# Youncy-Hu/MAGE

Hardware: AMD Instinct MI355X
Metric: generated frames/sec (64x64, 16-frame clips) (higher is better)
Workload: dtype bf16

## Files before the change

### __graft_entry__.py

```python
import os
import subprocess
import sys

ROOT = os.path.dirname(os.path.abspath(__file__))
if ROOT not in sys.path:
    sys.path.insert(0, ROOT)


def build() -> None:
    env = dict(os.environ)
    env.setdefault("HIPCC", "/opt/rocm/bin/hipcc")
    subprocess.run(["make", "-C", os.path.join(ROOT, "mage_amd", "csrc"), "-j4"], check=True, env=env)
    subprocess.run(["make", "-C", os.path.join(ROOT, "mage_amd", "csrc"), "check4"], check=True, env=env)
    import mage_amd
    from mage_amd import _lib
    lib = _lib.load()
    assert lib.mage_abi_version() == _lib.ABI_VERSION


def smoke() -> None:
    import torch
    from mage_amd.utils import synth
    from mage_amd.utils.util import instantiate_from_config
    from oracle import mage_oracle as O

    assert torch.cuda.is_available(), "smoke() needs a GPU"
    L, B, seed = 4, 2, 21
    cfg = synth.mnist_model_config(frames_length=L)
    model = instantiate_from_config(cfg).eval()
    synth.fill_state_dict(model, seed)
    sd = {k: v.detach().clone() for k, v in model.state_dict().items()}
    batch = synth.synth_batch_mnist(B, L, seed=seed)
    model = model.to("cuda:0")
    video = model.autoregressive_generate({k: v.to("cuda:0") for k, v in batch.items()})
    torch.cuda.synchronize()
    want, want_tok, _, trace = O.mage_generate(sd, batch, L, return_trace=True)
    err = (video.cpu() - want).abs().max().item()
    got_tok = model.last_tokens.cpu()
    tok_ok = torch.equal(got_tok, want_tok)
    top2 = trace.topk(2, dim=-1)[0]
    margin = (top2[..., 0] - top2[..., 1]).abs()
    bad = got_tok != want_tok
    n_soft, n_hard = int((bad & (margin <= 2e-5)).sum()), int((bad & (margin > 2e-5)).sum())
    print(f"smoke: video {tuple(video.shape)} max|d| vs oracle {err:.2e}, tokens bit-exact: {tok_ok} "
          f"(soft flips inside 2e-5 margin: {n_soft}, hard mismatches: {n_hard}, min margin {margin.min().item():.2e})")
    assert err < 1e-4 and n_hard == 0 and n_soft == 0 and tok_ok, "smoke: the HIP path left the oracle's tokens / frames"
    with open("/proc/self/maps") as f:
        assert "libmage_hip.so" in f.read(), "native library not loaded"


if __name__ == "__main__":
    build()
    if "--smoke" in sys.argv:
        smoke()
```

### include/mage_hip.h

```cpp
#ifndef MAGE_HIP_H
#define MAGE_HIP_H

#include <stdint.h>

#ifdef __cplusplus
extern "C" {
#endif

#define MAGE_ABI_VERSION 10

enum { MAGE_F32 = 0, MAGE_BF16 = 1, MAGE_BF16X3 = 2, MAGE_F16X3 = 3, MAGE_F16 = 4 };
enum { MAGE_OK = 0, MAGE_EINVAL = -1, MAGE_EHIP = -2, MAGE_EUNSUPPORTED = -3 };
enum { MAGE_ACT_NONE = 0, MAGE_ACT_RELU = 1, MAGE_ACT_QUICKGELU = 2, MAGE_ACT_GELU_ERF = 3, MAGE_ACT_TANH = 4,
       MAGE_ACT_QUICKGELU_GRAD = 5  };

int mage_abi_version(void);
const char* mage_last_error(void);
int mage_init(int device);
int mage_check_device_errors(void* stream);

int mage_set_option(const char* name, int32_t value);
int mage_get_option(const char* name, int32_t* value);

typedef struct mage_gemm_desc {
    int32_t dtype;
    int32_t M, N, K;
    const void* A;
    const void* W;
    void* Y;
    int32_t lda, ldy;
    int32_t y_dtype;
    int32_t out_h, out_w, in_h, in_w;
    int32_t a_img_stride, a_off;
    int32_t taps_h, taps_w, cin, stride;
    int32_t dy0, dx0, dys, dxs;
    int32_t y_img_stride, y_mul_y, y_mul_x, y_off;
    const float* bias;
    const float* scale;
    const float* shift;
    int32_t act;
    const float* rowadd;
    int32_t rowadd_div, rowadd_mod;
    const void* residual;
    int32_t ldr, res_dtype;
    int32_t post_relu;
    int32_t ldw;
    int32_t n_split;
    int64_t a_split_stride, w_split_stride, y_split_stride;
    void* y2;
    int32_t ldy2;
    int32_t res_half;
    float* ln_part;
    const float* ln_stats;
    const float* ln_colsum;
    int32_t a_half;
    float ln_eps;
    const void* head_w;
    int32_t head_phases;
    int32_t a_relu;
    int64_t ln_part_rows;
} mage_gemm_desc;

int mage_gemm(const mage_gemm_desc* desc, void* stream);
int mage_gemm_kernel_name(const mage_gemm_desc* desc, char* buf, int32_t len);
int mage_gemm_is_small(int32_t M, int32_t N, int32_t K);
int mage_ln_stats(const float* part, int64_t rows, int32_t n_slices, int32_t C, float eps, float* stats, void* stream);
int mage_row_stats(const void* x, int32_t dtype, int64_t rows, int32_t C, int64_t ldx, float eps, float* stats, void* stream);

int mage_split(const float* x, int64_t ldx, void* y, int64_t ldy, int64_t rows, int32_t C, int32_t kind, void* stream);

int mage_split_rows(const float* x, int64_t ldx, void* y, int64_t rows, int32_t C, int32_t kind, int32_t relu, int64_t group,
                    int64_t group_stride, int64_t off, int64_t inner, int64_t inner_stride, float* x_relu, void* stream);

int mage_layernorm(const float* x, const float* gamma, const float* beta, void* y, int32_t y_dtype,
                   int64_t rows, int32_t C, float eps, void* stream);

typedef struct mage_attn_desc {
    int32_t dtype;
    const void* q;
    const void* k;
    const void* v;
    void* out;
    int32_t ldq, ldk, ldv, ldo;
    int32_t n_seq, inner;
    int32_t nq, nk, n_head;
    int32_t q_outer_stride, q_axis_stride;
    int32_t kv_outer_stride, kv_axis_stride;
    int32_t causal;
    const int32_t* kv_len;
    int32_t kv_len_div;
    float scale;
    int32_t out_split;
    float drop_p;
    uint64_t drop_seed;
    int32_t o_outer_stride, o_axis_stride;
} mage_attn_desc;

int mage_attention(const mage_attn_desc* desc, void* stream);

int mage_embedding(const int64_t* ids, const float* table, void* out, int32_t out_dtype, int64_t n,
                   int32_t C, int32_t n_table, int32_t relu, int64_t group, int64_t group_stride, int64_t off,
                   int64_t inner, int64_t inner_stride, void* stream);

int mage_table_conv(const int64_t* ids, int64_t n_img, int32_t H, int32_t W, int32_t taps_h, int32_t taps_w, const void* table,
                    int32_t table_dtype, int32_t n_codes, int32_t C, const float* pos, const float* bias, int32_t relu, const float* rowadd,
                    int64_t rowadd_div, int32_t rowadd_mod, void* y, int32_t y_dtype, int64_t ldy, int64_t group, int64_t y_group_stride,
                    int64_t y_off, void* stream);

int mage_resblock_table(const int64_t* ids, int64_t n_img, int32_t H, int32_t W, const void* table, int32_t n_codes, int32_t C,
                        const float* bias3, const float* codebook, const void* w1, const float* b1, const float* scale1, const float* shift1,
                        int32_t post_relu, void* y, int64_t ldy, int64_t y_img_stride, int64_t y_row_pitch, int64_t y_off, void* stream);

int mage_resblock_rows(const void* t, int64_t lda, const void* w1, const float* b1, const float* scale1, const float* shift1,
                       const void* residual, int64_t ldr, int32_t post_relu, void* y, int64_t ldy, int64_t n_img, int32_t H, int32_t W,
                       int32_t C, int64_t img_stride, int64_t row_pitch, int64_t off, void* stream);

int mage_vq_nearest(const float* z, const float* codebook_t, const float* c2, int64_t M, int32_t D, int32_t K,
                    int64_t* idx, float* margin, void* stream);
int mage_vq_prepare(const float* codebook, int32_t K, int32_t D, float* codebook_t, float* c2, void* stream);

int mage_argmax(const float* logits, int64_t rows, int32_t K, int64_t ld, int64_t group, int64_t in_group_stride,
                int64_t in_off, int64_t* out, int64_t out_group_stride, int64_t out_off, float* margin, void* stream);

#define MAGE_SAMPLE_MAX_K 4096
int mage_sample_tokens(const float* logits, int64_t rows, int32_t K, int64_t ld, int64_t group, int64_t in_group_stride,
                       int64_t in_off, int64_t* out, int64_t out_group_stride, int64_t out_off, const int64_t* seeds,
                       int64_t pos_off, float temperature, int32_t top_k, float top_p, void* stream);

int mage_token_logprob(const float* logits, int64_t rows, int32_t K, int64_t ld, int64_t group, int64_t in_group_stride, int64_t in_off,
                       const int64_t* tokens, float* logprob, int64_t tok_group_stride, int64_t tok_off, void* stream);

int mage_clip_scores(const float* logprob, int64_t n_clips, int32_t n_cand, int64_t per_clip, float* scores, int64_t* best, void* stream);

int mage_cross_entropy(const float* logits, const int64_t* target, int64_t rows, int32_t K, float* row_loss,
                       float* loss_mean, void* stream);

int mage_conv_in(const float* x, const float* weight_t, const float* bias, const float* scale, const float* shift,
                 void* y, int32_t y_dtype, int32_t N, int32_t cin, int32_t H, int32_t W, int32_t cout,
                 int32_t kh, int32_t kw, int32_t stride, int32_t pad, int32_t act, int32_t s2d, void* stream);
int mage_conv_out(const void* x, int32_t x_dtype, const float* weight_t, const float* bias, float* y,
                  int32_t N, int32_t IH, int32_t IW, int32_t cin, int32_t cout, int32_t transposed, void* stream);
int mage_convt_fold_tanh(const float* taps, const float* bias, float* y, int32_t N, int32_t IH, int32_t IW,
                         int32_t cout, void* stream);

int mage_maxpool2(const void* x, void* y, int32_t dtype, int32_t N, int32_t H, int32_t W, int32_t C, int32_t relu,
                  void* stream);
int mage_upsample2(const void* x, void* y, int32_t dtype, int32_t N, int32_t H, int32_t W, int32_t C, void* stream);
int mage_relu(const void* x, void* y, int32_t dtype, int64_t n, void* stream);
int mage_cast(const void* x, int32_t x_dtype, void* y, int32_t y_dtype, int64_t n, void* stream);

int mage_adain(const float* x, const float* gamma, const float* beta, float* out, int32_t B, int32_t P, int32_t C,
               float eps, void* stream);

int mage_add_scaled_rowvec(float* x, const float* s, const float* vec, int32_t B, int32_t P, int32_t C, void* stream);

int mage_row_affine(float* x, const float* rs, const float* table, int64_t rows, int32_t C, int32_t div, int32_t mod,
                    void* stream);

int mage_caption_mask(const int64_t* ids, int32_t B, int32_t S, int64_t padding_idx, int32_t* kv_len, float* keep, void* stream);
int mage_copy2d(void* dst, int64_t dst_pitch, const void* src, int64_t src_pitch, int64_t width_bytes, int64_t height, void* stream);

int mage_groupnorm_silu(const float* x, int64_t sample_stride_rows, int64_t row_off, int32_t n_samples, int32_t rows_per_sample,
                        int32_t C, int32_t groups, const float* gamma, const float* beta, float eps, float* stats, void* y,
                        int32_t y_dtype, void* stream);

int mage_groupnorm_act(const float* x, int64_t sample_stride_rows, int64_t row_off, int32_t n_samples, int32_t rows_per_sample,
                       int32_t C, int32_t groups, const float* gamma, const float* beta, float eps, float* stats,
                       const float* residual, int32_t act, void* y, int32_t y_dtype, int64_t y_sample_stride_rows,
                       int64_t y_row_off, void* stream);

int mage_reparam_kl(const float* mu, const float* logvar, const float* eps, float* out, float* kl_sum, int32_t B, int64_t n,
                    void* stream);

int mage_mse(const float* a, int64_t lda, const float* b, int64_t ldb, int64_t rows, int32_t cols, double* workspace, float* out,
             void* stream);



int mage_transpose(const void* x, int32_t dtype, int64_t ldx, void* y, int64_t ldy, int64_t y_row0, int64_t M, int64_t Mp, int32_t C,
                   int32_t out_h, int32_t out_w, int32_t in_h, int32_t in_w, int64_t img_stride, int64_t a_off, int32_t dy, int32_t dx,
                   int32_t stride, void* stream);
int mage_transpose_colsum(const void* x, int64_t ldx, void* y, int64_t ldy, int64_t M, int64_t Mp, int32_t C, int32_t out_w,
                          int64_t img_stride, int64_t a_off, float* colsum, int32_t n_part, void* stream);
int mage_gemm_tn(const void* dY, int64_t lda, const void* X, int64_t ldb, int64_t T, int32_t N, int32_t K, int32_t n_split,
                 int64_t tokens_per_split, float* partials, float* db_partials, void* stream);
int mage_colsum(const void* x, int64_t ld, int64_t T, int32_t C, float* partials, int32_t n_part, void* stream);
int mage_row_sum(const void* x, int32_t dtype, int64_t ld, int64_t n, int32_t rows, float* out, int32_t n_chunk, void* stream);
int mage_sum_partials(const float* part, int64_t stride, int32_t n_part, int64_t n, float* out, int32_t accumulate, void* stream);
int mage_layernorm_bwd(const float* x, const float* gamma, const void* dy, int32_t dy_dtype, float* dx, float* partials, int32_t n_part,
                       int64_t rows, int32_t C, float eps, int32_t accumulate, void* dx_bf16, float p, uint64_t seed, void* stream);
int mage_act(const void* x, void* y, int32_t dtype, int64_t n, int32_t act, void* stream);
int mage_act_bwd(const void* x, const void* dy, void* dx, int32_t dtype, int64_t n, int32_t act, void* stream);
int mage_cross_entropy_bwd(const float* logits, const int64_t* target, int64_t rows, int32_t K, const float* grad_out, void* dlogits,
                           int32_t dl_dtype, void* stream);
int mage_embedding_bwd(const int64_t* ids, const void* dout, int32_t dout_dtype, float* dtable, int64_t n, int32_t C, int32_t n_table,
                       int64_t padding_idx, int64_t group, int64_t group_stride, int64_t off, float* scratch, int64_t scratch_floats,
                       void* stream);
int mage_group_rowsum(const void* x, int32_t dtype, int64_t rows, int32_t C, int64_t div, int64_t mod, const float* row_scale,
                      int64_t row_scale_div, float* out, int32_t n_chunk, void* stream);
int mage_attention_bwd(const mage_attn_desc* desc, const void* dout, void* dq, void* dk, void* dv, int32_t ld_dq, int32_t ld_dk,
                       int32_t ld_dv, void* stream);
int mage_dropout(const void* x, int32_t x_dtype, void* y, int32_t y_dtype, int64_t n, float p, uint64_t seed, int32_t accumulate,
                 void* stream);
int mage_dropout_add(const void* x, int32_t x_dtype, const float* r, float* y, void* y_bf16, int64_t n, float p, uint64_t seed, void* stream);
int mage_dropout_add_layernorm(const void* x, int32_t x_dtype, const float* r, float* y, const float* gamma, const float* beta, void* yn,
                               int32_t yn_dtype, int64_t rows, int32_t C, float eps, float p, uint64_t seed, void* stream);
int mage_bn_colreduce(int32_t mode, const float* x, const float* dy, const float* mask, const float* mean, const float* rstd, int64_t rows,
                      int32_t C, float* partials, int32_t n_part, void* stream);
int mage_bn_apply(const float* x, const float* mean, const float* rstd, const float* gamma, const float* beta, const float* residual, void* y,
                  int32_t y_dtype, int64_t rows, int32_t C, int32_t relu, void* stream);
int mage_bn_bwd_apply(const float* x, const float* dy, const float* mask, const float* mean, const float* rstd, const float* gamma,
                      const float* sums, float* dx, int64_t rows, int32_t C, void* stream);
int mage_convt_unfold_tanh_bwd(const float* grad_y, const float* y, float* dtaps, int32_t N, int32_t IH, int32_t IW, int32_t cout, void* stream);
// ... 21 lines not shown
```

### mage_amd/_lib.py

```python
from __future__ import annotations

import ctypes as C
import os
from typing import Optional

_HERE = os.path.dirname(os.path.abspath(__file__))
LIB_PATH = os.environ.get("MAGE_HIP_LIB", os.path.join(_HERE, "lib", "libmage_hip.so"))

F32, BF16, BF16X3, F16X3, F16 = 0, 1, 2, 3, 4
ACT_NONE, ACT_RELU, ACT_QUICKGELU, ACT_GELU_ERF, ACT_TANH, ACT_QUICKGELU_GRAD = 0, 1, 2, 3, 4, 5
ABI_VERSION = 10

i32, i64, f32, vp = C.c_int32, C.c_int64, C.c_float, C.c_void_p


class GemmDesc(C.Structure):
    _fields_ = [
        ("dtype", i32), ("M", i32), ("N", i32), ("K", i32),
        ("A", vp), ("W", vp), ("Y", vp),
        ("lda", i32), ("ldy", i32), ("y_dtype", i32),
        ("out_h", i32), ("out_w", i32), ("in_h", i32), ("in_w", i32),
        ("a_img_stride", i32), ("a_off", i32),
        ("taps_h", i32), ("taps_w", i32), ("cin", i32), ("stride", i32),
        ("dy0", i32), ("dx0", i32), ("dys", i32), ("dxs", i32),
        ("y_img_stride", i32), ("y_mul_y", i32), ("y_mul_x", i32), ("y_off", i32),
        ("bias", vp), ("scale", vp), ("shift", vp),
        ("act", i32),
        ("rowadd", vp), ("rowadd_div", i32), ("rowadd_mod", i32),
        ("residual", vp), ("ldr", i32), ("res_dtype", i32),
        ("post_relu", i32), ("ldw", i32), ("n_split", i32),
        ("a_split_stride", i64), ("w_split_stride", i64), ("y_split_stride", i64),
        ("y2", vp), ("ldy2", i32), ("res_half", i32), ("ln_part", vp), ("ln_stats", vp), ("ln_colsum", vp), ("a_half", i32), ("ln_eps", C.c_float),
        ("head_w", vp), ("head_phases", i32), ("a_relu", i32), ("ln_part_rows", i64),
    ]


class AttnDesc(C.Structure):
    _fields_ = [
        ("dtype", i32), ("q", vp), ("k", vp), ("v", vp), ("out", vp),
        ("ldq", i32), ("ldk", i32), ("ldv", i32), ("ldo", i32),
        ("n_seq", i32), ("inner", i32), ("nq", i32), ("nk", i32), ("n_head", i32),
        ("q_outer_stride", i32), ("q_axis_stride", i32), ("kv_outer_stride", i32), ("kv_axis_stride", i32),
        ("causal", i32), ("kv_len", vp), ("kv_len_div", i32), ("scale", f32), ("out_split", i32), ("drop_p", f32), ("drop_seed", C.c_uint64),
        ("o_outer_stride", i32), ("o_axis_stride", i32),
    ]


SIGNATURES = {
    "mage_abi_version": (C.c_int, []),
    "mage_last_error": (C.c_char_p, []),
    "mage_init": (C.c_int, [C.c_int]),
    "mage_check_device_errors": (C.c_int, [vp]),
    "mage_set_option": (C.c_int, [C.c_char_p, i32]),
    "mage_get_option": (C.c_int, [C.c_char_p, C.POINTER(i32)]),
    "mage_gemm": (C.c_int, [C.POINTER(GemmDesc), vp]),
    "mage_gemm_kernel_name": (C.c_int, [C.POINTER(GemmDesc), C.c_char_p, i32]),
    "mage_gemm_is_small": (C.c_int, [i32, i32, i32]),
    "mage_ln_stats": (C.c_int, [vp, i64, i32, i32, f32, vp, vp]),
    "mage_row_stats": (C.c_int, [vp, i32, i64, i32, i64, f32, vp, vp]),
    "mage_groupnorm_bwd": (C.c_int, [vp, i64, i64, i32, i32, i32, i32, vp, vp, vp, vp, i32, vp, i64, i64, vp, vp, vp, vp, vp, vp]),
    "mage_adain_bwd": (C.c_int, [vp, vp, vp, vp, vp, i32, i32, i32, f32, vp]),
    "mage_reparam_kl_bwd": (C.c_int, [vp, vp, vp, vp, vp, vp, vp, i64, vp]),
    "mage_mse_bwd": (C.c_int, [vp, i64, vp, i64, i64, i32, vp, vp, i64, vp]),
    "mage_transpose_colsum": (C.c_int, [vp, i64, vp, i64, i64, i64, i32, i32, i64, i64, vp, i32, vp]),
    "mage_maxpool2_bwd": (C.c_int, [vp, vp, vp, i32, i32, i32, i32, vp]),
    "mage_upsample2_bwd": (C.c_int, [vp, vp, i32, i32, i32, i32, vp]),
    "mage_layernorm": (C.c_int, [vp, vp, vp, vp, i32, i64, i32, f32, vp]),
    "mage_split": (C.c_int, [vp, i64, vp, i64, i64, i32, i32, vp]),
    "mage_attention": (C.c_int, [C.POINTER(AttnDesc), vp]),
    "mage_embedding": (C.c_int, [vp, vp, vp, i32, i64, i32, i32, i32, i64, i64, i64, i64, i64, vp]),
    "mage_table_conv": (C.c_int, [vp, i64, i32, i32, i32, i32, vp, i32, i32, i32, vp, vp, i32, vp, i64, i32, vp, i32, i64, i64, i64, i64, vp]),
    "mage_resblock_table": (C.c_int, [vp, i64, i32, i32, vp, i32, i32, vp, vp, vp, vp, vp, vp, i32, vp, i64, i64, i64, i64, vp]),
    "mage_resblock_rows": (C.c_int, [vp, i64, vp, vp, vp, vp, vp, i64, i32, vp, i64, i64, i32, i32, i32, i64, i64, i64, vp]),
    "mage_vq_nearest": (C.c_int, [vp, vp, vp, i64, i32, i32, vp, vp, vp]),
    "mage_vq_prepare": (C.c_int, [vp, i32, i32, vp, vp, vp]),
    "mage_argmax": (C.c_int, [vp, i64, i32, i64, i64, i64, i64, vp, i64, i64, vp, vp]),
    "mage_sample_tokens": (C.c_int, [vp, i64, i32, i64, i64, i64, i64, vp, i64, i64, vp, i64, f32, i32, f32, vp]),
    "mage_token_logprob": (C.c_int, [vp, i64, i32, i64, i64, i64, i64, vp, vp, i64, i64, vp]),
    "mage_clip_scores": (C.c_int, [vp, i64, i32, i64, vp, vp, vp]),
    "mage_cross_entropy": (C.c_int, [vp, vp, i64, i32, vp, vp, vp]),
    "mage_conv_in": (C.c_int, [vp, vp, vp, vp, vp, vp, i32, i32, i32, i32, i32, i32, i32, i32, i32, i32, i32, i32, vp]),
    "mage_split_rows": (C.c_int, [vp, i64, vp, i64, i32, i32, i32, i64, i64, i64, i64, i64, vp, vp]),
    "mage_conv_out": (C.c_int, [vp, i32, vp, vp, vp, i32, i32, i32, i32, i32, i32, vp]),
    "mage_convt_fold_tanh": (C.c_int, [vp, vp, vp, i32, i32, i32, i32, vp]),
    "mage_maxpool2": (C.c_int, [vp, vp, i32, i32, i32, i32, i32, i32, vp]),
    "mage_upsample2": (C.c_int, [vp, vp, i32, i32, i32, i32, i32, vp]),
    "mage_relu": (C.c_int, [vp, vp, i32, i64, vp]),
    "mage_cast": (C.c_int, [vp, i32, vp, i32, i64, vp]),
    "mage_adain": (C.c_int, [vp, vp, vp, vp, i32, i32, i32, f32, vp]),
    "mage_add_scaled_rowvec": (C.c_int, [vp, vp, vp, i32, i32, i32, vp]),
    "mage_row_affine": (C.c_int, [vp, vp, vp, i64, i32, i32, i32, vp]),
    "mage_caption_mask": (C.c_int, [vp, i32, i32, i64, vp, vp, vp]),
    "mage_copy2d": (C.c_int, [vp, i64, vp, i64, i64, i64, vp]),
    "mage_groupnorm_silu": (C.c_int, [vp, i64, i64, i32, i32, i32, i32, vp, vp, f32, vp, vp, i32, vp]),
    "mage_groupnorm_act": (C.c_int, [vp, i64, i64, i32, i32, i32, i32, vp, vp, f32, vp, vp, i32, vp, i32, i64, i64, vp]),
    "mage_reparam_kl": (C.c_int, [vp, vp, vp, vp, vp, i32, i64, vp]),
    "mage_mse": (C.c_int, [vp, i64, vp, i64, i64, i32, vp, vp, vp]),
    "mage_transpose": (C.c_int, [vp, i32, i64, vp, i64, i64, i64, i64, i32, i32, i32, i32, i32, i64, i64, i32, i32, i32, vp]),
    "mage_bn_colreduce": (C.c_int, [i32, vp, vp, vp, vp, vp, i64, i32, vp, i32, vp]),
    "mage_bn_apply": (C.c_int, [vp, vp, vp, vp, vp, vp, vp, i32, i64, i32, i32, vp]),
    "mage_bn_bwd_apply": (C.c_int, [vp, vp, vp, vp, vp, vp, vp, vp, i64, i32, vp]),
    "mage_convt_unfold_tanh_bwd": (C.c_int, [vp, vp, vp, i32, i32, i32, i32, vp]),
    "mage_gemm_tn": (C.c_int, [vp, i64, vp, i64, i64, i32, i32, i32, i64, vp, vp, vp]),
    "mage_colsum": (C.c_int, [vp, i64, i64, i32, vp, i32, vp]),
    "mage_row_sum": (C.c_int, [vp, i32, i64, i64, i32, vp, i32, vp]),
    "mage_sum_partials": (C.c_int, [vp, i64, i32, i64, vp, i32, vp]),
    "mage_layernorm_bwd": (C.c_int, [vp, vp, vp, i32, vp, vp, i32, i64, i32, f32, i32, vp, f32, C.c_uint64, vp]),
    "mage_act": (C.c_int, [vp, vp, i32, i64, i32, vp]),
    "mage_act_bwd": (C.c_int, [vp, vp, vp, i32, i64, i32, vp]),
    "mage_cross_entropy_bwd": (C.c_int, [vp, vp, i64, i32, vp, vp, i32, vp]),
    "mage_embedding_bwd": (C.c_int, [vp, vp, i32, vp, i64, i32, i32, i64, i64, i64, i64, vp, i64, vp]),
    "mage_group_rowsum": (C.c_int, [vp, i32, i64, i32, i64, i64, vp, i64, vp, i32, vp]),
    "mage_attention_bwd": (C.c_int, [C.POINTER(AttnDesc), vp, vp, vp, vp, i32, i32, i32, vp]),
    "mage_dropout": (C.c_int, [vp, i32, vp, i32, i64, f32, C.c_uint64, i32, vp]),
    "mage_dropout_add": (C.c_int, [vp, i32, vp, vp, vp, i64, f32, C.c_uint64, vp]),
    "mage_dropout_add_layernorm": (C.c_int, [vp, i32, vp, vp, vp, vp, vp, i32, i64, i32, f32, f32, C.c_uint64, vp]),
    "mage_adam": (C.c_int, [vp, vp, vp, vp, i64, f32, f32, f32, f32, i32, f32, vp]),
}

_lib: Optional[C.CDLL] = None
_inited_devices = set()


class MageHipError(RuntimeError):
    pass


def load(path: str = LIB_PATH) -> C.CDLL:
    global _lib
    if _lib is not None:
        return _lib
    if not os.path.exists(path):
        raise MageHipError(
            f"{path} not found: the HIP extension is not built. Run `python -c 'import __graft_entry__ as g; g.build()'` "
            f"(or `make -C mage_amd/csrc`). There is no CPU/PyTorch fallback for the MAGE product path.")
    import torch
    lib = C.CDLL(path)
    for name, (res, args) in SIGNATURES.items():
        fn = getattr(lib, name)
        fn.restype, fn.argtypes = res, args
    if lib.mage_abi_version() != ABI_VERSION:
        raise MageHipError(f"libmage_hip.so ABI {lib.mage_abi_version()} != binding ABI {ABI_VERSION}: rebuild")
    _lib = lib
    return lib


def lib(device_index: int = 0) -> C.CDLL:
    l = load()
    if device_index not in _inited_devices:
        check(l.mage_init(int(device_index)), l)
        _inited_devices.add(device_index)
    return l


def check(code: int, l: Optional[C.CDLL] = None) -> None:
    if code == 0:
        return
    l = l or load()
    msg = (l.mage_last_error() or b"").decode(errors="replace")
    if code == -1:
        raise ValueError(f"mage_hip: {msg}")
    raise MageHipError(f"mage_hip error {code}: {msg}")
```

### mage_amd/config.py

```python
from __future__ import annotations

import contextlib
import dataclasses
import os
from typing import Iterator

__all__ = ["Config", "ENV", "get", "override", "lib_option", "lib_options", "lib_flag", "LIB_OPTIONS"]


@dataclasses.dataclass(frozen=True)
class Config:
    ln_fold: bool = True
    stream_16bit: bool = True
    attn_split: bool = True
    frame_table: bool = True
    auto_graph: bool = True
    encode_split: bool = True
    decode_table: bool = True
    decode_split: bool = True
    decode_taps8: bool = True
    decode_resblock_fusion: bool = True
    decode_head_fusion: bool = True
    decode_phase_merge: bool = True
    decode_relu_fold: bool = True
    train_f32_branch: bool = False
    train_wgrad_transpose: bool = False
    train_emit: bool = True
    train_dual: bool = True
    train_taps: bool = True
    train_enc_split: bool = True


ENV = {
    "ln_fold": ("MAGE_NO_LN_FOLD", False),
    "stream_16bit": ("MAGE_STREAM_FP32", False),
    "attn_split": ("MAGE_ATTN_SPLIT_FP32", False),
    "frame_table": ("MAGE_NO_FRAME_TABLE", False),
    "auto_graph": ("MAGE_NO_AUTO_GRAPH", False),
    "encode_split": ("MAGE_ENCODE_FP32", False),
    "decode_table": ("MAGE_NO_DECODE_TABLE", False),
    "decode_split": ("MAGE_DECODE_FP32", False),
    "decode_taps8": ("MAGE_DECODE_NO_TAPS8", False),
    "decode_resblock_fusion": ("MAGE_DECODE_NO_RESBLOCK_FUSION", False),
    "decode_head_fusion": ("MAGE_DECODE_NO_HEAD_FUSION", False),
    "decode_phase_merge": ("MAGE_DECODE_NO_PHASE_MERGE", False),
    "decode_relu_fold": ("MAGE_DECODE_NO_RELU_FOLD", False),
    "train_f32_branch": ("MAGE_TRAIN_F32_BRANCH", True),
    "train_wgrad_transpose": ("MAGE_WGRAD_TRANSPOSE", True),
    "train_emit": ("MAGE_TRAIN_NO_EMIT", False),
    "train_dual": ("MAGE_TRAIN_NO_DUAL", False),
    "train_taps": ("MAGE_TRAIN_NO_TAPS", False),
    "train_enc_split": ("MAGE_TRAIN_ENC_FP32", False),
}

LIB_OPTIONS = ("gemm_no_4w", "gemm_no_4h", "gemm_4h_plain", "gemm4_train_forms", "gemm_no_8phase", "gemm_no_taps8", "gemm_no_narrow", "gemm_no_narrow_few", "gemm_no_small",
               "gemm_small_m", "gemm_stagger_groups", "gemm_stagger_percent", "gemm_stagger_forced",
               "gemm4_stagger_groups", "gemm4_stagger_percent", "attn_no_mfma", "attn_no_fewq", "vq_no_mfma", "conv_no_tile")


def _set(v) -> bool:
    return bool(v) and v != "0"


def _from_env() -> Config:
    kw = {}
    for field, (var, when_set) in ENV.items():
        if _set(os.environ.get(var)):
            kw[field] = when_set
    return Config(**kw)


_CONFIG = _from_env()


def get() -> Config:
    return _CONFIG


@contextlib.contextmanager
def override(**kw) -> Iterator[Config]:
    global _CONFIG
    saved = _CONFIG
    _CONFIG = dataclasses.replace(saved, **kw)
    try:
        yield _CONFIG
    finally:
        _CONFIG = saved


_LIB_CACHE = None


def invalidate_lib_options() -> None:
    global _LIB_CACHE
    _LIB_CACHE = None


def _lib_cache() -> dict:
    global _LIB_CACHE
    if _LIB_CACHE is None:
        import ctypes as C
        from . import _lib
        l = _lib.load()
        out = {}
        for name in LIB_OPTIONS:
            v = C.c_int32(0)
            _lib.check(l.mage_get_option(name.encode(), C.byref(v)), l)
            out[name] = int(v.value)
        _LIB_CACHE = out
    return _LIB_CACHE


def lib_options() -> dict:
    return dict(_lib_cache())


def lib_flag(name: str) -> int:
    c = _lib_cache()
    if name not in c:
        raise KeyError(f"unknown library option '{name}' (mage_amd.config.LIB_OPTIONS)")
    return c[name]


def set_lib_option(name: str, value: int) -> None:
    from . import _lib
    l = _lib.load()
    try:
        _lib.check(l.mage_set_option(name.encode(), int(value)), l)
    finally:
        invalidate_lib_options()


@contextlib.contextmanager
def lib_option(name: str, value: int) -> Iterator[None]:
    old = lib_flag(name)
    set_lib_option(name, value)
    try:
        yield
    finally:
        set_lib_option(name, old)
```

### mage_amd/csrc/common.h

```cpp
#pragma once
#include <hip/hip_runtime.h>
#include <stdint.h>
#include <stdio.h>
#include <stdarg.h>
#include "../../include/mage_hip.h"

typedef __bf16 bf16_t;
typedef __attribute__((ext_vector_type(8))) __bf16 bf16x8;
typedef __attribute__((ext_vector_type(4))) __bf16 bf16x4;
typedef __attribute__((ext_vector_type(4))) float f32x4;
typedef __attribute__((ext_vector_type(4))) unsigned int u32x4;

#define MAGE_MAX_DEVICES 16
void mage_set_error(const char* fmt, ...);
int mage_device_index();
const void* mage_zero_page();
int* mage_error_word();
enum { MAGE_DEVERR_EMBEDDING_ID = 1, MAGE_DEVERR_CE_TARGET = 2, MAGE_DEVERR_TOKEN_ID = 3 };
struct MageOptions {
    int gemm_no_4w;
    int gemm_no_4h;
    int gemm_4h_plain;
    int gemm4_train_forms;
    int gemm_no_8phase;
    int gemm_no_taps8;
    int gemm_no_narrow;
    int gemm_no_narrow_few;
    int gemm_no_small;
    int gemm_small_m;
    int gemm_stagger_groups, gemm_stagger_percent, gemm_stagger_forced;
    int gemm4_stagger_groups, gemm4_stagger_percent;
    int attn_no_mfma;
    int attn_no_fewq;
    int vq_no_mfma;
    int conv_no_tile;
};
const MageOptions& mage_options();
__device__ __forceinline__ void mage_raise(int* word, int code, long value, int bound) {
    if (atomicCAS(word, 0, code) == 0) {
        word[1] = (int)value;
        word[2] = bound;
    }
}

#if defined(MAGE_DEBUG) && MAGE_DEBUG
#include <cassert>
#define MAGE_DASSERT(cond) assert(cond)
#else
#define MAGE_DASSERT(cond) ((void)0)
#endif

#define MAGE_CHECK_ARG(cond, ...)                                   \
    do {                                                            \
        if (!(cond)) {                                              \
            mage_set_error(__VA_ARGS__);                            \
            return MAGE_EINVAL;                                     \
        }                                                           \
    } while (0)

#define MAGE_CHECK_LAUNCH(name)                                                         \
    do {                                                                                \
        hipError_t e_ = hipGetLastError();                                              \
        if (e_ != hipSuccess) {                                                         \
            mage_set_error("%s: launch failed: %s", name, hipGetErrorString(e_));       \
            return MAGE_EHIP;                                                           \
        }                                                                               \
    } while (0)

int mage_gemm_cu_count();
extern thread_local const void** mage_gemm_plan;
template <auto KERNEL, typename Args>
int mage_gemm_launch(unsigned grid, unsigned block, unsigned lds, hipStream_t s, const Args& a) {
    if (mage_gemm_plan) {
        *mage_gemm_plan = (const void*)KERNEL;
        return MAGE_OK;
    }
    static bool attr[MAGE_MAX_DEVICES] = {false};
    const int dev = mage_device_index();
    MAGE_CHECK_ARG(dev >= 0, "mage_gemm: no current device");
    if (!attr[dev]) {
        (void)hipFuncSetAttribute((const void*)KERNEL, hipFuncAttributeMaxDynamicSharedMemorySize, lds);
        attr[dev] = true;
    }
    hipLaunchKernelGGL(KERNEL, dim3(grid), dim3(block), lds, s, a);
    MAGE_CHECK_LAUNCH("mage_gemm");
    return MAGE_OK;
}

__device__ __forceinline__ unsigned short f2bf_bits(float f) {
    unsigned int u = __float_as_uint(f);
    if ((u & 0x7fffffffu) > 0x7f800000u) return (unsigned short)((u >> 16) | 0x40);
    u += 0x7fffu + ((u >> 16) & 1u);
    return (unsigned short)(u >> 16);
}
__device__ __forceinline__ float bf_bits2f(unsigned short b) { return __uint_as_float(((unsigned int)b) << 16); }

template <typename T> __device__ __forceinline__ float to_f32(T v);
template <> __device__ __forceinline__ float to_f32<float>(float v) { return v; }
template <> __device__ __forceinline__ float to_f32<unsigned short>(unsigned short v) { return bf_bits2f(v); }

template <typename T> __device__ __forceinline__ T from_f32(float v);
template <> __device__ __forceinline__ float from_f32<float>(float v) { return v; }
template <> __device__ __forceinline__ unsigned short from_f32<unsigned short>(float v) { return f2bf_bits(v); }

typedef _Float16 f16_t;
template <> __device__ __forceinline__ float to_f32<f16_t>(f16_t v) { return (float)v; }
template <> __device__ __forceinline__ f16_t from_f32<f16_t>(float v) { return (f16_t)v; }

__device__ __forceinline__ f32x4 load4(const float* p) { return *(const f32x4*)p; }
__device__ __forceinline__ f32x4 load4(const unsigned short* p) {
    uint2 r = *(const uint2*)p;
    f32x4 o;
    o[0] = __uint_as_float(r.x << 16);
    o[1] = __uint_as_float(r.x & 0xffff0000u);
    o[2] = __uint_as_float(r.y << 16);
    o[3] = __uint_as_float(r.y & 0xffff0000u);
    return o;
}
__device__ __forceinline__ void store4(float* p, f32x4 v) { *(f32x4*)p = v; }
__device__ __forceinline__ void mage_ln_stats_row(const float2* __restrict__ p, long stride, int n_slices, float inv_c, float eps, float& mean, float& rstd) {
    float s1 = 0.f, s2 = 0.f;
    for (int i = 0; i < n_slices; ++i) {
        const float2 v = p[(long)i * stride];
        s1 = __fadd_rn(s1, v.x);
        s2 = __fadd_rn(s2, v.y);
    }
    mean = __fmul_rn(s1, inv_c);
    const float var = fmaxf(__fmaf_rn(-mean, mean, __fmul_rn(s2, inv_c)), 0.f);
    rstd = __fdiv_rn(1.0f, __fsqrt_rn(__fadd_rn(var, eps)));
}

typedef __attribute__((ext_vector_type(2))) __bf16 bf16x2_t;
__device__ __forceinline__ unsigned int pack_bf16x2(float a, float b) {
    bf16x2_t v = {(__bf16)a, (__bf16)b};
    return __builtin_bit_cast(unsigned int, v);
}
__device__ __forceinline__ void store4(unsigned short* p, f32x4 v) {
    uint2 r;
    r.x = pack_bf16x2(v[0], v[1]);
    r.y = pack_bf16x2(v[2], v[3]);
    *(uint2*)p = r;
}

__device__ __forceinline__ void store8(unsigned short* p, f32x4 a, f32x4 b) {
    uint4 r;
    r.x = pack_bf16x2(a[0], a[1]);
    r.y = pack_bf16x2(a[2], a[3]);
    r.z = pack_bf16x2(b[0], b[1]);
    r.w = pack_bf16x2(b[2], b[3]);
    *(uint4*)p = r;
}
__device__ __forceinline__ void store8(float* p, f32x4 a, f32x4 b) { *(f32x4*)p = a; *(f32x4*)(p + 4) = b; }

typedef __attribute__((ext_vector_type(2))) _Float16 f16x2_t;
typedef __attribute__((ext_vector_type(8))) _Float16 f16x8;
__device__ __forceinline__ unsigned int pack_f16x2(float a, float b) {
    const f16x2_t v = {(_Float16)a, (_Float16)b};
    return __builtin_bit_cast(unsigned int, v);
}
__device__ __forceinline__ float2 unpack_f16x2(unsigned int u) {
    const f16x2_t v = __builtin_bit_cast(f16x2_t, u);
    return float2{(float)v[0], (float)v[1]};
}
__device__ __forceinline__ float2 unpack_bf16x2(unsigned int u) { return float2{__uint_as_float(u << 16), __uint_as_float(u & 0xffff0000u)}; }
template <typename T> __device__ __forceinline__ unsigned int pack16x2(float a, float b) {
    if constexpr (sizeof(T) == 2 && !__is_same(T, unsigned short)) return pack_f16x2(a, b);
    else return pack_bf16x2(a, b);
}
template <typename T> __device__ __forceinline__ float2 unpack16x2(unsigned int u) {
    if constexpr (sizeof(T) == 2 && !__is_same(T, unsigned short)) return unpack_f16x2(u);
    else return unpack_bf16x2(u);
}
template <typename T> __device__ __forceinline__ f32x4 widen4(uint2 r) {
    const float2 a = unpack16x2<T>(r.x), b = unpack16x2<T>(r.y);
    return f32x4{a.x, a.y, b.x, b.y};
}
template <typename T> __device__ __forceinline__ f32x4 mfma16x16x32(const u32x4& a, const u32x4& b, const f32x4& c) {
    if constexpr (sizeof(T) == 2 && !__is_same(T, unsigned short))
        return __builtin_amdgcn_mfma_f32_16x16x32_f16(__builtin_bit_cast(f16x8, a), __builtin_bit_cast(f16x8, b), c, 0, 0, 0);
    else
        return __builtin_amdgcn_mfma_f32_16x16x32_bf16(__builtin_bit_cast(bf16x8, a), __builtin_bit_cast(bf16x8, b), c, 0, 0, 0);
}
__device__ __forceinline__ f32x4 load4(const f16_t* p) { return widen4<f16_t>(*(const uint2*)p); }
__device__ __forceinline__ void store4(f16_t* p, f32x4 v) { *(uint2*)p = uint2{pack_f16x2(v[0], v[1]), pack_f16x2(v[2], v[3])}; }
__device__ __forceinline__ void store8(f16_t* p, f32x4 a, f32x4 b) {
    *(uint4*)p = uint4{pack_f16x2(a[0], a[1]), pack_f16x2(a[2], a[3]), pack_f16x2(b[0], b[1]), pack_f16x2(b[2], b[3])};
// ... 72 lines not shown
```

### mage_amd/csrc/gemm.hip

```cpp
#include <cxxabi.h>
#include <cstring>
#include <mutex>
#include <string>
#include <unordered_map>
#include "gemm_impl.h"

int mage_gemm_f16(const mage_gemm_desc* d, hipStream_t s);

#ifdef MAGE_PROBE
extern "C" int mage_debug_read_waves(void* dst, size_t bytes) {
    return hipMemcpyFromSymbol(dst, HIP_SYMBOL(mage_probe_wave), bytes < sizeof(mage_probe_wave) ? bytes : sizeof(mage_probe_wave)) ==
                   hipSuccess
               ? 0
               : -1;
}
extern "C" int mage_debug_read_seg(void* dst, size_t bytes) {
    return hipMemcpyFromSymbol(dst, HIP_SYMBOL(mage_probe_seg), bytes < sizeof(mage_probe_seg) ? bytes : sizeof(mage_probe_seg)) ==
                   hipSuccess
               ? 0
               : -1;
}
extern "C" int mage_debug_read(void* dst, size_t bytes) {
    return hipMemcpyFromSymbol(dst, HIP_SYMBOL(mage_probe_buf), bytes < sizeof(mage_probe_buf) ? bytes : sizeof(mage_probe_buf)) ==
                   hipSuccess
               ? 0
               : -1;
}
#endif


extern "C" int mage_gemm_is_small(int32_t M, int32_t N, int32_t K) {
    MAGE_CHECK_ARG(mage_device_index() >= 0 && M > 0 && N > 0 && K > 0, "mage_gemm_is_small: no current device / bad sizes");
    return small_shape(M, N, K, mage_gemm_cu_count()) ? 1 : 0;
}

extern "C" int mage_gemm(const mage_gemm_desc* d_in, void* stream) {
    MAGE_CHECK_ARG(d_in != nullptr, "mage_gemm: null descriptor");
    mage_gemm_desc dn = *d_in;
    const bool spl = dn.dtype == MAGE_BF16X3 || dn.dtype == MAGE_F16X3;
    if (dn.ldw == 0) dn.ldw = spl ? 2 * dn.K : dn.K;
    if (dn.n_split <= 0) dn.n_split = 1;
    const mage_gemm_desc* d = &dn;
    MAGE_CHECK_ARG(d->ldw >= (spl ? 2 * d->K : d->K), "mage_gemm: ldw=%d < K=%d", d->ldw, d->K);
    MAGE_CHECK_ARG(d->ldw == d->K || d->n_split > 1 || spl,
                   "mage_gemm: ldw=%d != K=%d: a W row stride other than K is read only by the split-K (n_split > 1) and split-precision forms", d->ldw, d->K);
    MAGE_CHECK_ARG(mage_zero_page() != nullptr, "mage_gemm: mage_init() has not been called");
    const bool h16 = d->dtype == MAGE_F16;
    MAGE_CHECK_ARG(d->dtype == MAGE_F32 || d->dtype == MAGE_BF16 || h16 || spl, "mage_gemm: bad dtype %d", d->dtype);
    MAGE_CHECK_ARG(d->y_dtype == MAGE_F32 || (d->y_dtype == MAGE_BF16 && !h16) || ((spl || h16) && d->y_dtype == d->dtype),
                   "mage_gemm: bad y_dtype %d for dtype %d (fp32, or the operands' 16-bit / split type; fp32 operands may write bf16)", d->y_dtype, d->dtype);
    MAGE_CHECK_ARG(!d->residual || d->res_dtype == MAGE_F32 || (d->res_dtype == MAGE_BF16 && !h16) || (h16 && d->res_dtype == MAGE_F16),
                   "mage_gemm: bad res_dtype %d for dtype %d", d->res_dtype, d->dtype);
    MAGE_CHECK_ARG(!spl || (d->K % 64 == 0 && d->cin % 64 == 0 && d->lda >= 2 * d->cin && d->y_dtype != MAGE_BF16),
                   "mage_gemm: split-precision operands need K and cin multiples of 64, lda >= 2 cin (16-bit elements), fp32 or split output");
    MAGE_CHECK_ARG(!spl || d->y_dtype == MAGE_F32 || (d->N % 64 == 0 && d->ldy % 8 == 0 && d->ldy >= 2 * d->N && (((uintptr_t)d->Y) & 255) == 0),
                   "mage_gemm: split output needs N %% 64 == 0, ldy >= 2N (16-bit elements), Y 256-byte aligned");
    MAGE_CHECK_ARG(d->M > 0 && d->N > 0 && d->K > 0, "mage_gemm: empty problem M=%d N=%d K=%d", d->M, d->N, d->K);
    MAGE_CHECK_ARG(d->A && d->W && d->Y, "mage_gemm: null operand");
    const int ch = d->dtype == MAGE_F32 ? 4 : 8;
    MAGE_CHECK_ARG(d->N % 8 == 0, "mage_gemm: N=%d must be a multiple of 8", d->N);
    MAGE_CHECK_ARG(d->K % ch == 0 && d->lda % ch == 0 && d->cin % ch == 0,
                   "mage_gemm: K=%d, lda=%d, cin=%d must be multiples of %d", d->K, d->lda, d->cin, ch);
    MAGE_CHECK_ARG(d->ldy % 4 == 0 && (!d->residual || d->ldr % 4 == 0), "mage_gemm: ldy/ldr must be multiples of 4");
    MAGE_CHECK_ARG((d->y_dtype != MAGE_BF16 && d->y_dtype != MAGE_F16) || d->ldy % 8 == 0, "mage_gemm: 16-bit output needs ldy a multiple of 8 (16-byte accesses)");
    MAGE_CHECK_ARG(!d->residual || d->res_dtype == MAGE_F32 || d->ldr % 8 == 0, "mage_gemm: a 16-bit residual needs ldr a multiple of 8 (16-byte accesses)");
    MAGE_CHECK_ARG(d->taps_h >= 1 && d->taps_w >= 1 && d->K == d->taps_h * d->taps_w * d->cin,
                   "mage_gemm: K=%d != taps_h*taps_w*cin = %d*%d*%d", d->K, d->taps_h, d->taps_w, d->cin);
    MAGE_CHECK_ARG(d->out_h >= 1 && d->out_w >= 1 && d->in_h >= 1 && d->in_w >= 1, "mage_gemm: bad geometry");
    MAGE_CHECK_ARG(!d->scale == !d->shift, "mage_gemm: scale and shift must be given together");
    MAGE_CHECK_ARG(!d->rowadd || (d->rowadd_div >= 1 && d->rowadd_mod >= 1), "mage_gemm: bad rowadd div/mod");
    MAGE_CHECK_ARG((((uintptr_t)d->A | (uintptr_t)d->W | (uintptr_t)d->Y) & 15) == 0, "mage_gemm: operands must be 16-byte aligned");
    const bool gather_ = d->taps_h * d->taps_w > 1 || d->stride != 1 || d->dy0 != 0 || d->dx0 != 0 || d->in_h != d->out_h || d->in_w != d->out_w;
    MAGE_CHECK_ARG(d->n_split == 1 || (!gather_ && !d->residual && !d->rowadd && !d->scale && !d->post_relu && !d->bias &&
                                       d->out_h == 1 && d->out_w >= d->M && d->act == MAGE_ACT_NONE),
                   "mage_gemm: n_split > 1 is the plain split-K form (no gather, no epilogue extras, rows not regrouped)");
    MAGE_CHECK_ARG(d->n_split == 1 || ((d->a_split_stride | d->w_split_stride) % ch == 0 && d->y_split_stride % 4 == 0 && d->ldw % ch == 0),
                   "mage_gemm: split strides / ldw must keep 16-byte alignment");
    hipStream_t s = (hipStream_t)stream;
    MAGE_CHECK_ARG(!d->a_half || (d->in_h % 2 == 0 && d->in_w % 2 == 0 && d->n_split == 1), "mage_gemm: a_half needs an even in_h x in_w grid");
    MAGE_CHECK_ARG(!d->res_half || (d->residual && d->out_h > 1 && d->out_h % 2 == 0 && d->out_w % 2 == 0 && d->n_split == 1),
                   "mage_gemm: res_half needs a residual and an even out_h x out_w output plane");
    MAGE_CHECK_ARG(!d->ln_part || d->ln_part_rows > (d->ln_colsum ? (int64_t)d->M - 1 : (int64_t)(d->M - 1) * d->y_mul_x + d->y_off),
                   "mage_gemm: ln_part needs ln_part_rows (rows of the slice-major partial-sum buffer) > the largest row it is indexed with");
    MAGE_CHECK_ARG(!d->a_relu || (d->dtype == MAGE_BF16 && !gather_ && !d->a_half && d->N <= 128 && d->n_split == 1 && !d->residual && !d->rowadd && !d->scale &&
                                  !d->post_relu && !d->y2 && !d->ln_part && !d->ln_stats && !d->ln_colsum && !d->head_w),
                   "mage_gemm: a_relu is a form of the bf16 plain GEMM with N <= 128 (epilogue act(acc + bias) only)");
    if (spl) {
        const bool tapsform = gather_ || d->rowadd;
        MAGE_CHECK_ARG(!d->head_w, "mage_gemm: head_w is a fusion of the bf16 padded-taps form");
        if (tapsform) {
            const int r = d->dtype == MAGE_BF16X3 ? try_taps8<1>(d, s) : try_taps8<2>(d, s);
            if (r) return r < 0 ? r : MAGE_OK;
            mage_set_error("mage_gemm: split-precision form: this convolution / row-table geometry is not eligible for the padded-taps kernel");
            return MAGE_EUNSUPPORTED;
        }
        return d->dtype == MAGE_BF16X3 ? launch_spl<1>(d, s) : launch_spl<2>(d, s);
    }
    if (h16) {
        MAGE_CHECK_ARG(!d->head_w && d->n_split == 1 && !d->scale && !d->post_relu && !d->res_half && !d->a_half,
                       "mage_gemm: MAGE_F16 operands do not take head_w / n_split / scale+shift / post_relu / res_half / a_half");
        return mage_gemm_f16(d, s);
    }
    if (const int r = try_taps8(d, s)) return r < 0 ? r : MAGE_OK;
    MAGE_CHECK_ARG(!d->head_w, "mage_gemm: head_w is a fusion of the bf16 padded-taps form; this geometry does not run there");
    if (const int r = mage_conv3x3_c64_try(d, s)) return r < 0 ? r : MAGE_OK;
    if (const int r = mage_gemm4_try(d, s)) return r < 0 ? r : MAGE_OK;
    const bool gather = d->taps_h * d->taps_w > 1 || d->stride != 1 || d->dy0 != 0 || d->dx0 != 0 || d->in_h != d->out_h ||
                        d->in_w != d->out_w || d->a_half;
    if (d->dtype == MAGE_BF16) return gather ? launch<MAGE_BF16, true>(d, s) : launch<MAGE_BF16, false>(d, s);
    return gather ? launch<MAGE_F32, true>(d, s) : launch<MAGE_F32, false>(d, s);
}

thread_local const void** mage_gemm_plan = nullptr;

extern "C" int mage_gemm_kernel_name(const mage_gemm_desc* desc, char* buf, int32_t len) {
    MAGE_CHECK_ARG(buf != nullptr && len > 0, "mage_gemm_kernel_name: no buffer");
    const void* kernel = nullptr;
    mage_gemm_plan = &kernel;
    const int r = mage_gemm(desc, nullptr);
    mage_gemm_plan = nullptr;
    if (r != MAGE_OK) return r;
    static std::mutex mu;
    static std::unordered_map<const void*, std::string> names;
    std::string name;
    {
        std::lock_guard<std::mutex> lock(mu);
        auto it = names.find(kernel);
        if (it == names.end()) {
            hipFunction_t f = nullptr;
            const char* raw = hipGetFuncBySymbol(&f, kernel) == hipSuccess ? hipKernelNameRef(f) : nullptr;
            if (!raw) {
                mage_set_error("mage_gemm_kernel_name: the runtime has no name for the selected kernel");
                return MAGE_EHIP;
            }
            std::string n = raw;
            int status = -1;
            if (char* dm = n.compare(0, 2, "_Z") == 0 ? abi::__cxa_demangle(raw, nullptr, nullptr, &status) : nullptr) {
                if (status == 0) n = dm;
                free(dm);
            }
            for (const char* drop : {"void ", "(anonymous namespace)::"})
                for (size_t at; (at = n.find(drop)) != std::string::npos;) n.erase(at, strlen(drop));
            n = n.substr(0, n.find('('));
            it = names.emplace(kernel, n).first;
        }
        name = it->second;
    }
    MAGE_CHECK_ARG((int32_t)name.size() < len, "mage_gemm_kernel_name: %d bytes are too few for '%s'", (int)len, name.c_str());
    memcpy(buf, name.c_str(), name.size() + 1);
    return MAGE_OK;
}
```

### mage_amd/csrc/gemm_shared.h

```cpp
#pragma once
#include <type_traits>
#include "common.h"

namespace {

__device__ __forceinline__ void glds16(const void* src, char* lds_wave_base) {
    __builtin_amdgcn_global_load_lds((const __attribute__((address_space(1))) void*)src,
                                     (__attribute__((address_space(3))) void*)lds_wave_base, 16, 0, 0);
}

template <int ACT>
__device__ __forceinline__ float act_apply(float v) {
    if (ACT == MAGE_ACT_RELU) return fmaxf(v, 0.f);
    if (ACT == MAGE_ACT_QUICKGELU) return v * __builtin_amdgcn_rcpf(1.f + __builtin_amdgcn_exp2f(-2.4554669596f * v));
    if (ACT == MAGE_ACT_GELU_ERF) return 0.5f * v * (1.f + erff(v * 0.70710678118654752f));
    return v;
}

enum { EK_BIAS = 0, EK_RES_INIT = 1, EK_GENERAL = 2 };

struct LnConsume {
    float mean[8], rstd[8];
    f32x4 s[4];
};
enum { LN_NONE = 0, LN_PRODUCE = 1, LN_CONSUME = 2, LN_DUAL = 3, LN_GELUBWD = 4, LN_HEAD = 5 };

template <int ACT, typename OT, int MT, bool AFFINE = false, int LN = LN_NONE, int OSPL = 0,
          typename HT = std::conditional_t<sizeof(OT) == 2, OT, unsigned short>, bool RESE = false>
__device__ __forceinline__ void epilogue_lean(const mage_gemm_desc& d, const f32x4 (&bias)[4], f32x4 (&acc)[MT][4], int m0, int n0,
                                              int lane, int plane, char* stg, long ysplit, const LnConsume* lnc = nullptr) {
    constexpr bool F32 = sizeof(OT) == 4;
    static_assert((LN != LN_DUAL && LN != LN_GELUBWD) || std::is_same<HT, unsigned short>::value, "training forms: bf16 rows");
    static_assert(!RESE || (sizeof(OT) == 2 && OSPL == 0 && (LN == LN_NONE || LN == LN_PRODUCE)), "residual in the epilogue: 16-bit rows out");
    constexpr int RB = F32 ? 256 : 128;
    constexpr int NCH = RB / 16;
    constexpr int RPI = 64 / NCH;
    constexpr int NST = 16 / RPI;
    constexpr int CPC = 16 / (int)sizeof(OT);
    const int l15 = lane & 15, grp = lane >> 4;
    int woff[4];
#pragma unroll
    for (int nt = 0; nt < 4; ++nt)
        woff[nt] = OSPL ? l15 * RB + (((nt * 2 + (grp >> 1)) ^ l15) << 4) + (grp & 1) * 8
                 : F32  ? l15 * RB + (((nt * 4 + grp) ^ l15) << 4)
                        : l15 * RB + (((nt * 2 + (grp >> 1)) ^ ((l15 >> 1) & 7)) << 4) + (grp & 1) * 8;
    const int rr = lane / NCH, cc = lane % NCH;
    int roff[NST];
#pragma unroll
    for (int i = 0; i < NST; ++i) {
        const int r = rr + RPI * i;
        roff[i] = F32 ? r * RB + ((cc ^ r) << 4) : r * RB + ((cc ^ ((r >> 1) & 7)) << 4);
    }
    const int col = n0 + cc * CPC;
#pragma unroll
    for (int nt = 0; nt < 4; ++nt)
        MAGE_DASSERT(woff[nt] >= 0 && (OSPL ? (woff[nt] | 128) + 8 : woff[nt] + (F32 ? 16 : 8)) <= 4096);
#pragma unroll
    for (int i = 0; i < NST; ++i) MAGE_DASSERT(roff[i] >= 0 && roff[i] + 16 <= 4096);
    const bool simple_rows = d.out_h == 1 && d.out_w >= d.M;
    const bool affine_rows = AFFINE && d.out_h == 1 && d.y_mul_x == 1 && d.out_w % 256 == 0;
    const bool interior = (simple_rows || affine_rows) && m0 + MT * 16 <= d.M && n0 + 64 <= d.N;
    const bool cv_ok = col < d.N;
    const long row_shift = (AFFINE && !simple_rows && affine_rows) ? (long)(m0 / d.out_w) * (d.y_img_stride - d.out_w) : 0;
    const int ldy = OSPL ? d.ldy >> 1 : d.ldy;
    OT* yp = (OT*)d.Y + ysplit + ((long)((m0 + rr) * d.y_mul_x + d.y_off) + row_shift) * ldy + col;
    const long step = (long)RPI * d.y_mul_x * ldy;
    [[maybe_unused]] HT* y2p = nullptr;
    [[maybe_unused]] long step2 = 0;
    if constexpr (LN == LN_PRODUCE) {
        y2p = (HT*)d.y2 + (long)((m0 + rr) * d.y_mul_x + d.y_off) * d.ldy2 + col;
        step2 = (long)RPI * d.y_mul_x * d.ldy2;
    }

    [[maybe_unused]] u32x4 auxr[2][2];
    [[maybe_unused]] auto aux_request = [&](int mt) {
        const unsigned short* ap = (const unsigned short*)d.y2 + (long)((m0 + mt * 16 + (lane >> 3)) * d.y_mul_x + d.y_off) * d.ldy2 + n0 + (lane & 7) * 8;
#pragma unroll
        for (int i = 0; i < 2; ++i) auxr[mt & 1][i] = *(const u32x4*)(ap + (long)(8 * i) * d.y_mul_x * d.ldy2);
    };
    if constexpr (LN == LN_GELUBWD) aux_request(0);
    constexpr int RD = 3;
    [[maybe_unused]] u32x4 rland[RESE ? RD : 1][2];
    [[maybe_unused]] const HT* rbase = nullptr;
    [[maybe_unused]] auto res_request = [&](int t) {
#pragma unroll
        for (int i = 0; i < 2; ++i) {
            const int m = min(m0 + t * 16 + (lane >> 3) + 8 * i, d.M - 1);
            if constexpr (AFFINE) {
                const int img = m / plane, rem = m - img * plane;
                const int oy = rem / d.out_w, ox = rem - oy * d.out_w;
                const long rrow = d.res_half ? (long)img * (plane >> 2) + (long)(oy >> 1) * (d.out_w >> 1) + (ox >> 1) : (long)m;
                rland[t % RD][i] = *(const u32x4*)(rbase + rrow * d.ldr);
            } else {
                rland[t % RD][i] = *(const u32x4*)(rbase + (long)(m * d.y_mul_x + d.y_off) * d.ldr);
            }
        }
    };
    if constexpr (RESE) {
        const int rcol = n0 + (lane & 7) * 8;
        rbase = (const HT*)d.residual + (rcol < d.N ? rcol : 0);
#pragma unroll
        for (int t = 0; t < RD && t < MT; ++t) res_request(t);
    }
    auto stage = [&](int mt, u32x4 (&o)[NST], auto apply_act) {
        [[maybe_unused]] float s1 = 0.f, s2 = 0.f;
        [[maybe_unused]] uint2 auxb[4];
        if constexpr (RESE) {
#pragma unroll
            for (int i = 0; i < 2; ++i) {
                const int r = (lane >> 3) + 8 * i;
                *(u32x4*)(stg + 2048 + r * 128 + (((lane & 7) ^ ((r >> 1) & 7)) << 4)) = rland[mt % RD][i];
            }
            if (mt + RD < MT) res_request(mt + RD);
#pragma unroll
            for (int nt = 0; nt < 4; ++nt)
                auxb[nt] = *(const uint2*)(stg + 2048 + l15 * 128 + (((nt * 2 + (grp >> 1)) ^ ((l15 >> 1) & 7)) << 4) + (grp & 1) * 8);
        }
        if constexpr (LN == LN_GELUBWD) {
            if (mt + 1 < MT) aux_request(mt + 1);
#pragma unroll
            for (int i = 0; i < 2; ++i) {
                const int r = (lane >> 3) + 8 * i;
                *(u32x4*)(stg + 2048 + r * 128 + (((lane & 7) ^ ((r >> 1) & 7)) << 4)) = auxr[mt & 1][i];
            }
#pragma unroll
            for (int nt = 0; nt < 4; ++nt)
                auxb[nt] = *(const uint2*)(stg + 2048 + l15 * 128 + (((nt * 2 + (grp >> 1)) ^ ((l15 >> 1) & 7)) << 4) + (grp & 1) * 8);
        }
#pragma unroll
        for (int nt = 0; nt < 4; ++nt) {
            f32x4 v;
            if constexpr (LN == LN_CONSUME) v = (acc[mt][nt] - lnc->s[nt] * lnc->mean[mt]) * lnc->rstd[mt] + bias[nt];
            else v = acc[mt][nt] + bias[nt];
            if constexpr (RESE) v = v + widen4<HT>(auxb[nt]);
            if constexpr (LN == LN_PRODUCE) {
                s1 += (v[0] + v[1]) + (v[2] + v[3]);
                s2 += (v[0] * v[0] + v[1] * v[1]) + (v[2] * v[2] + v[3] * v[3]);
            }
            if constexpr (LN == LN_GELUBWD) {
                const uint2 ax = auxb[nt];
                const f32x4 x = f32x4{__uint_as_float(ax.x << 16), __uint_as_float(ax.x & 0xffff0000u), __uint_as_float(ax.y << 16),
                                      __uint_as_float(ax.y & 0xffff0000u)};
                const f32x4 t = x * -2.4554669596f;
                f32x4 sg;
#pragma unroll
                for (int e = 0; e < 4; ++e) sg[e] = __builtin_amdgcn_rcpf(1.0f + __builtin_amdgcn_exp2f(t[e]));
                v = v * (sg * (1.0f + (x * 1.702f) * (1.0f - sg)));
            }
            if constexpr (!decltype(apply_act)::value) {
            } else if constexpr (ACT == MAGE_ACT_QUICKGELU) {
                const f32x4 t = v * -2.4554669596f;
                f32x4 e4;
#pragma unroll
                for (int e = 0; e < 4; ++e) e4[e] = __builtin_amdgcn_exp2f(t[e]);
                e4 = e4 + 1.0f;
#pragma unroll
                for (int e = 0; e < 4; ++e) e4[e] = __builtin_amdgcn_rcpf(e4[e]);
                v = v * e4;
            } else if (ACT != MAGE_ACT_NONE) {
#pragma unroll
                for (int e = 0; e < 4; ++e) v[e] = act_apply<ACT>(v[e]);
            }
            if constexpr (OSPL != 0) {
                uint2 hi, lo;
                split_pack2<OSPL>(v[0], v[1], hi.x, lo.x);
                split_pack2<OSPL>(v[2], v[3], hi.y, lo.y);
                *(uint2*)(stg + woff[nt]) = hi;
                *(uint2*)(stg + (woff[nt] ^ 128)) = lo;
            } else if constexpr (F32) {
                *(f32x4*)(stg + woff[nt]) = v;
            } else {
                *(uint2*)(stg + woff[nt]) = uint2{pack16x2<OT>(v[0], v[1]), pack16x2<OT>(v[2], v[3])};
            }
        }
        if constexpr (LN == LN_PRODUCE) {
            s1 += __shfl_xor(s1, 16);
            s2 += __shfl_xor(s2, 16);
            s1 += __shfl_xor(s1, 32);
            s2 += __shfl_xor(s2, 32);
            if (grp == 0) {
                const long row = (long)(m0 + mt * 16 + l15) * d.y_mul_x + d.y_off;
                float* pp = d.ln_part + ((long)(n0 >> 6) * d.ln_part_rows + row) * 2;
                *(float2*)pp = float2{s1, s2};
            }
        }
#pragma unroll
        for (int i = 0; i < NST; ++i) o[i] = *(const u32x4*)(stg + roff[i]);
    };
    auto store = [&](int mt, const u32x4 (&o)[NST]) {
#pragma unroll
        for (int i = 0; i < NST; ++i) {
            if (interior) {
#ifdef MAGE_EPI_NO_STORE
                asm volatile("" ::"v"(o[i]), "v"(yp));
#else
#ifdef MAGE_EPI_PLAIN_STORE
                *(u32x4*)yp = o[i];
#else
                __builtin_nontemporal_store(o[i], (u32x4*)yp);
#endif
#endif
                yp += step;
                if constexpr (LN == LN_PRODUCE && F32) {
                    const uint2 pk = uint2{pack16x2<HT>(__uint_as_float(o[i][0]), __uint_as_float(o[i][1])),
                                           pack16x2<HT>(__uint_as_float(o[i][2]), __uint_as_float(o[i][3]))};
                    typedef unsigned u32x2_t __attribute__((ext_vector_type(2)));
                    __builtin_nontemporal_store(u32x2_t{pk.x, pk.y}, (u32x2_t*)y2p);
                    y2p += step2;
                }
            } else {
                const int m = m0 + mt * 16 + rr + RPI * i;
                if (m < d.M && cv_ok) {
                    int yrow;
                    if (simple_rows) {
                        yrow = m * d.y_mul_x + d.y_off;
                    } else {
                        const int img = m / plane;
                        const int rem = m - img * plane;
                        const int oy = rem / d.out_w;
                        const int ox = rem - oy * d.out_w;
                        yrow = img * d.y_img_stride + oy * d.y_mul_y + ox * d.y_mul_x + d.y_off;
                    }
                    __builtin_nontemporal_store(o[i], (u32x4*)((OT*)d.Y + ysplit + (long)yrow * ldy + col));
                }
            }
        }
    };
    if constexpr (LN == LN_DUAL) {
        OT* yp2 = (OT*)d.y2 + (long)((m0 + rr) * d.y_mul_x + d.y_off) * d.ldy2 + col;
        const long step2d = (long)RPI * d.y_mul_x * d.ldy2;
        u32x4 oa[NST], ob[NST];
#pragma unroll
        for (int mt = 0; mt < MT; ++mt) {
            stage(mt, oa, std::false_type{});
            stage(mt, ob, std::true_type{});
#pragma unroll
            for (int i = 0; i < NST; ++i) {
                __builtin_nontemporal_store(oa[i], (u32x4*)yp);
                yp += step;
                __builtin_nontemporal_store(ob[i], (u32x4*)yp2);
                yp2 += step2d;
            }
        }
        return;
    }
    u32x4 o[2][NST];
    stage(0, o[0], std::true_type{});
#pragma unroll
    for (int mt = 0; mt < MT; ++mt) {
        if (mt + 1 < MT) stage(mt + 1, o[(mt + 1) & 1], std::true_type{});
        store(mt, o[mt & 1]);
    }
}


__device__ __forceinline__ void ring_barrier() {
    asm volatile("" ::: "memory");
    __builtin_amdgcn_s_barrier();
    asm volatile("" ::: "memory");
}

}
```

### mage_amd/csrc/norm_attn.hip

```cpp
#include <cstdlib>
#include <type_traits>

#include "common.h"

namespace {

template <typename OT, int VPL>
__global__ __launch_bounds__(256) void layernorm_kernel(const float* __restrict__ x, const float* __restrict__ gamma,
                                                        const float* __restrict__ beta, OT* __restrict__ y, long rows,
                                                        int C, float eps) {
    const int lane = threadIdx.x & 63;
    const long row = (long)blockIdx.x * 4 + (threadIdx.x >> 6);
    if (row >= rows) return;
    const float* xr = x + row * C;
    f32x4 v[VPL];
    float s = 0.f;
#pragma unroll
    for (int j = 0; j < VPL; ++j) {
        const int c = j * 256 + lane * 4;
        v[j] = (c < C) ? *(const f32x4*)(xr + c) : f32x4{0.f, 0.f, 0.f, 0.f};
        s += (v[j][0] + v[j][1]) + (v[j][2] + v[j][3]);
    }
    const float mean = wave_sum(s) / (float)C;
    float q = 0.f;
#pragma unroll
    for (int j = 0; j < VPL; ++j) {
        const int c = j * 256 + lane * 4;
        if (c < C) {
#pragma unroll
            for (int e = 0; e < 4; ++e) {
                const float dlt = v[j][e] - mean;
                q += dlt * dlt;
            }
        }
    }
    const float rstd = 1.0f / sqrtf(wave_sum(q) / (float)C + eps);
    OT* yr = y + row * C;
#pragma unroll
    for (int j = 0; j < VPL; ++j) {
        const int c = j * 256 + lane * 4;
        if (c < C) {
            const f32x4 gm = *(const f32x4*)(gamma + c), bt = *(const f32x4*)(beta + c);
            f32x4 o;
#pragma unroll
            for (int e = 0; e < 4; ++e) o[e] = (v[j][e] - mean) * rstd * gm[e] + bt[e];
            store4(yr + c, o);
        }
    }
}

__device__ __forceinline__ void load8f(const float* p, f32x4& a, f32x4& b) {
    a = *(const f32x4*)p;
    b = *(const f32x4*)(p + 4);
}
__device__ __forceinline__ void load8f(const unsigned short* p, f32x4& a, f32x4& b) {
    const uint4 r = *(const uint4*)p;
    a = f32x4{__uint_as_float(r.x << 16), __uint_as_float(r.x & 0xffff0000u), __uint_as_float(r.y << 16), __uint_as_float(r.y & 0xffff0000u)};
    b = f32x4{__uint_as_float(r.z << 16), __uint_as_float(r.z & 0xffff0000u), __uint_as_float(r.w << 16), __uint_as_float(r.w & 0xffff0000u)};
}
__device__ __forceinline__ void copy8(const float* src, float* dst) {
    *(f32x4*)dst = *(const f32x4*)src;
    *(f32x4*)(dst + 4) = *(const f32x4*)(src + 4);
}
__device__ __forceinline__ void copy8(const unsigned short* src, unsigned short* dst) { *(uint4*)dst = *(const uint4*)src; }
__device__ __forceinline__ void load8f(const f16_t* p, f32x4& a, f32x4& b) {
    const uint4 r = *(const uint4*)p;
    a = widen4<f16_t>(uint2{r.x, r.y});
    b = widen4<f16_t>(uint2{r.z, r.w});
}
__device__ __forceinline__ void copy8(const f16_t* src, f16_t* dst) { *(uint4*)dst = *(const uint4*)src; }

template <typename T, int NK_MAX, typename OT = T>
__global__ __launch_bounds__(256) void attention_kernel(const mage_attn_desc d, int hg) {
    extern __shared__ __attribute__((aligned(16))) char smem_raw[];
    T* ks = (T*)smem_raw;
    const int rowf = hg * 32;
    T* vs = ks + (long)d.nk * rowf;
    const int s = blockIdx.x;
    const int h0 = blockIdx.y * hg;
    const int outer = s / d.inner, in = s - outer * d.inner;
    const long q_base = (long)outer * d.q_outer_stride + in;
    const long o_base = d.o_axis_stride ? (long)outer * d.o_outer_stride + in : q_base;
    const long o_step = d.o_axis_stride ? d.o_axis_stride : d.q_axis_stride;
    const long kv_base = (long)outer * d.kv_outer_stride + in;
    const T* kp = (const T*)d.k;
    const T* vp = (const T*)d.v;
    const int vec_per_row = rowf / 8;
    for (int e = threadIdx.x; e < d.nk * vec_per_row; e += 256) {
        const int j = e / vec_per_row, c = (e - j * vec_per_row) * 8;
        const long row = kv_base + (long)j * d.kv_axis_stride;
        copy8(kp + row * d.ldk + h0 * 32 + c, ks + j * rowf + c);
        copy8(vp + row * d.ldv + h0 * 32 + c, vs + j * rowf + c);
    }
    __syncthreads();
    int klen = d.nk;
    if (d.kv_len) klen = min(klen, d.kv_len[s / d.kv_len_div]);
    const unsigned drop_thresh = d.drop_p > 0.f ? (unsigned)((double)d.drop_p * 4294967296.0) : 0u;
    const float inv_keep = 1.0f / (1.0f - d.drop_p);
    const T* qp = (const T*)d.q;
    OT* op = (OT*)d.out;
    const int ldo = std::is_same<OT, T>::value ? d.ldo : d.ldo >> 1;
    for (int p = threadIdx.x; p < d.nq * hg; p += 256) {
        const int hl = p / d.nq, i = p - hl * d.nq;
        const long row = q_base + (long)i * d.q_axis_stride;
        f32x4 q[8];
#pragma unroll
        for (int c = 0; c < 4; ++c) {
            load8f(qp + row * d.ldq + (h0 + hl) * 32 + c * 8, q[2 * c], q[2 * c + 1]);
            q[2 * c] *= d.scale;
            q[2 * c + 1] *= d.scale;
        }
        const int jmax = d.causal ? min(klen, i + 1 + (d.nk - d.nq)) : klen;
        float sc[NK_MAX];
        float mx = -INFINITY;
#pragma unroll
        for (int j = 0; j < NK_MAX; ++j) {
            float a = -INFINITY;
            if (j < jmax) {
                const T* kr = ks + j * rowf + hl * 32;
                float a0 = 0.f, a1 = 0.f;
#pragma unroll
                for (int c = 0; c < 4; ++c) {
                    f32x4 k0, k1;
                    load8f(kr + c * 8, k0, k1);
                    a0 += q[2 * c][0] * k0[0] + q[2 * c][1] * k0[1] + q[2 * c][2] * k0[2] + q[2 * c][3] * k0[3];
                    a1 += q[2 * c + 1][0] * k1[0] + q[2 * c + 1][1] * k1[1] + q[2 * c + 1][2] * k1[2] + q[2 * c + 1][3] * k1[3];
                }
                a = a0 + a1;
            }
            sc[j] = a;
            mx = fmaxf(mx, a);
        }
        float den = 0.f;
        f32x4 o[8];
#pragma unroll
        for (int c = 0; c < 8; ++c) o[c] = f32x4{0.f, 0.f, 0.f, 0.f};
#pragma unroll
        for (int j = 0; j < NK_MAX; ++j) {
            if (j < jmax) {
                float pj = expf(sc[j] - mx);
                den += pj;
                if (drop_thresh) {
                    const unsigned long long idx = (((unsigned long long)s * d.n_head + (h0 + hl)) * d.nq + i) * d.nk + j;
                    pj = hash32(d.drop_seed * 0x9e3779b97f4a7c15ULL + idx) >= drop_thresh ? pj * inv_keep : 0.f;
                }
                const T* vr = vs + j * rowf + hl * 32;
#pragma unroll
                for (int c = 0; c < 4; ++c) {
                    f32x4 v0, v1;
                    load8f(vr + c * 8, v0, v1);
                    o[2 * c] += pj * v0;
                    o[2 * c + 1] += pj * v1;
                }
            }
        }
        const float inv = 1.0f / den;
        OT* orow = op + (o_base + (long)i * o_step) * ldo + (h0 + hl) * 32;
#pragma unroll
        for (int c = 0; c < 4; ++c) store8(orow + c * 8, o[2 * c] * inv, o[2 * c + 1] * inv);
    }
}

typedef __attribute__((ext_vector_type(8))) __bf16 abf16x8;
typedef __attribute__((ext_vector_type(4))) short ashort4;
typedef __attribute__((ext_vector_type(4))) _Float16 ahalf4;
template <typename HT> __device__ __forceinline__ void attn_p_split(float p, short& hi, short& lo) {
    if constexpr (std::is_same<HT, f16_t>::value) {
        const _Float16 h = (_Float16)p;
        hi = __builtin_bit_cast(short, h);
        lo = __builtin_bit_cast(short, (_Float16)(p - (float)h));
    } else {
        const unsigned hb = __float_as_uint(p) & 0xffff0000u;
        hi = (short)(hb >> 16);
        lo = (short)(__float_as_uint(p - __uint_as_float(hb)) >> 16);
    }
}
template <typename HT> __device__ __forceinline__ f32x4 attn_mfma_pv(const ashort4& vt, const ashort4& p, const f32x4& o) {
    if constexpr (std::is_same<HT, f16_t>::value)
        return __builtin_amdgcn_mfma_f32_16x16x16f16(__builtin_bit_cast(ahalf4, vt), __builtin_bit_cast(ahalf4, p), o, 0, 0, 0);
    else
        return __builtin_amdgcn_mfma_f32_16x16x16bf16_1k(vt, p, o, 0, 0, 0);
}
template <typename HT> __device__ __forceinline__ f32x4 attn_mfma_qk(const uint4& k, const uint4& q) {
    return mfma16x16x32<HT>(__builtin_bit_cast(u32x4, k), __builtin_bit_cast(u32x4, q), f32x4{0.f, 0.f, 0.f, 0.f});
}

template <int NKB, int MAXH, typename HT = unsigned short>
__global__ __launch_bounds__(256) void attention_mfma_kernel(const mage_attn_desc d) {
    extern __shared__ __attribute__((aligned(16))) char smem_raw[];
    unsigned short* vs = (unsigned short*)smem_raw;
    const int rowf = d.n_head * 32, vpitch = rowf + 16;
    const int s = blockIdx.x;
    const int outer = s / d.inner, in = s - outer * d.inner;
    const long q_base = (long)outer * d.q_outer_stride + in;
    const long o_base = d.o_axis_stride ? (long)outer * d.o_outer_stride + in : q_base;
    const long o_step = d.o_axis_stride ? d.o_axis_stride : d.q_axis_stride;
    const long kv_base = (long)outer * d.kv_outer_stride + in;
    const unsigned short* qp = (const unsigned short*)d.q;
    const unsigned short* kp = (const unsigned short*)d.k;
    const unsigned short* vp = (const unsigned short*)d.v;
    HT* op = (HT*)d.out;
    const int vec_per_row = rowf / 8;
    for (int e = threadIdx.x; e < 16 * NKB * vec_per_row; e += 256) {
        const int j = e / vec_per_row, c = (e - j * vec_per_row) * 8;
        uint4 val = uint4{0u, 0u, 0u, 0u};
        if (j < d.nk) val = *(const uint4*)(vp + (kv_base + (long)j * d.kv_axis_stride) * d.ldv + c);
        *(uint4*)(vs + j * vpitch + c) = val;
    }
    int klen = d.nk;
    if (d.kv_len) klen = min(klen, d.kv_len[s / d.kv_len_div]);
    const int lane = threadIdx.x & 63, wave = threadIdx.x >> 6;
    const int r = lane & 15, g = lane >> 4;
    uint4 kf[MAXH][NKB];
#pragma unroll
    for (int t = 0; t < MAXH; ++t) {
        const int h = wave + 4 * t;
        if (h < d.n_head) {
#pragma unroll
            for (int kb = 0; kb < NKB; ++kb) {
                const long krow = kv_base + (long)min(kb * 16 + r, d.nk - 1) * d.kv_axis_stride;
                kf[t][kb] = *(const uint4*)(kp + krow * d.ldk + h * 32 + g * 8);
            }
        }
    }
    __syncthreads();
    const int nqb = (d.nq + 15) >> 4;
    for (int qb = 0; qb < nqb; ++qb) {
        const int qi = qb * 16 + r;
        const long qrow = q_base + (long)min(qi, d.nq - 1) * d.q_axis_stride;
        const int jmax = d.causal ? min(klen, qi + 1 + (d.nk - d.nq)) : klen;
        uint4 qf[MAXH];
#pragma unroll
        for (int t = 0; t < MAXH; ++t) {
            const int h = wave + 4 * t;
            if (h < d.n_head) qf[t] = *(const uint4*)(qp + qrow * d.ldq + h * 32 + g * 8);
        }
#pragma unroll
        for (int t = 0; t < MAXH; ++t) {
            const int h = wave + 4 * t;
            if (h >= d.n_head) break;
            f32x4 st[NKB];
            float mx = -INFINITY;
#pragma unroll
            for (int kb = 0; kb < NKB; ++kb) {
                st[kb] = attn_mfma_qk<HT>(kf[t][kb], qf[t]);
#pragma unroll
                for (int e = 0; e < 4; ++e) {
                    st[kb][e] = (kb * 16 + 4 * g + e < jmax) ? st[kb][e] * d.scale : -INFINITY;
                    mx = fmaxf(mx, st[kb][e]);
                }
            }
            mx = fmaxf(mx, __shfl_xor(mx, 16));
            mx = fmaxf(mx, __shfl_xor(mx, 32));
            float den = 0.f;
            ashort4 phi[NKB], plo[NKB];
#pragma unroll
            for (int kb = 0; kb < NKB; ++kb)
#pragma unroll
                for (int e = 0; e < 4; ++e) {
                    const float p = (kb * 16 + 4 * g + e < jmax) ? expf(st[kb][e] - mx) : 0.f;
                    den += p;
                    short ph, pl;
                    attn_p_split<HT>(p, ph, pl);
                    phi[kb][e] = ph;
                    plo[kb][e] = pl;
                }
            den += __shfl_xor(den, 16);
            den += __shfl_xor(den, 32);
            f32x4 o[2];
#pragma unroll
            for (int b = 0; b < 2; ++b) {
                o[b] = f32x4{0.f, 0.f, 0.f, 0.f};
#pragma unroll
                for (int kb = 0; kb < NKB; ++kb) {
                    const unsigned short* vr = vs + (kb * 16 + 4 * g) * vpitch + h * 32 + b * 16 + r;
                    ashort4 vt;
#pragma unroll
                    for (int e = 0; e < 4; ++e) vt[e] = (short)vr[e * vpitch];
                    o[b] = attn_mfma_pv<HT>(vt, phi[kb], o[b]);
                    o[b] = attn_mfma_pv<HT>(vt, plo[kb], o[b]);
                }
            }
            const float inv = 1.0f / den;
            f32x4 v0, v1;
#pragma unroll
            for (int e = 0; e < 4; ++e) {
                const auto sw = __builtin_amdgcn_permlane16_swap(__float_as_uint(o[0][e]), __float_as_uint(o[1][e]), false, false);
                v0[e] = __uint_as_float(sw[0]) * inv;
                v1[e] = __uint_as_float(sw[1]) * inv;
            }
            if (qi < d.nq) {
                const int col = h * 32 + 16 * (g & 1) + 8 * (g >> 1);
                store8(op + (o_base + (long)qi * o_step) * d.ldo + col, v0, v1);
            }
        }
    }
}

template <int N> __device__ __forceinline__ float row_shr_f(float old, float src) {
    if constexpr (N == 0) return src;
    else return __uint_as_float(__builtin_amdgcn_update_dpp(__float_as_uint(old), __float_as_uint(src), 0x110 + N, 0xf, 0xf, false));
}
template <int N> __device__ __forceinline__ unsigned row_shl_u(unsigned src) {
    if constexpr (N == 0) return src;
    else return __builtin_amdgcn_update_dpp(src, src, 0x100 + N, 0xf, 0xf, false);
}
template <int N> __device__ __forceinline__ float row_shl_f(float src) { return __uint_as_float(row_shl_u<N>(__float_as_uint(src))); }
template <int N> __device__ __forceinline__ ashort4 row_shl_s4(ashort4 src) {
    const uint2 u = __builtin_bit_cast(uint2, src);
    return __builtin_bit_cast(ashort4, uint2{row_shl_u<N>(u.x), row_shl_u<N>(u.y)});
}

template <int NKB, typename HT = unsigned short>
__global__ __launch_bounds__(256) void attention_mfma_fewq_kernel(const mage_attn_desc d) {
    const int lane = threadIdx.x & 63;
    const int s = blockIdx.x * 4 + (threadIdx.x >> 6);
    if (s >= d.n_seq) return;
    const int outer = s / d.inner, in = s - outer * d.inner;
    const long q_base = (long)outer * d.q_outer_stride + in;
    const long o_base = d.o_axis_stride ? (long)outer * d.o_outer_stride + in : q_base;
    const long o_step = d.o_axis_stride ? d.o_axis_stride : d.q_axis_stride;
    const long kv_base = (long)outer * d.kv_outer_stride + in;
    const unsigned short* qp = (const unsigned short*)d.q;
    const unsigned short* kp = (const unsigned short*)d.k;
    const unsigned short* vp = (const unsigned short*)d.v;
    HT* op = (HT*)d.out;
    int klen = d.nk;
    if (d.kv_len) klen = min(klen, d.kv_len[s / d.kv_len_div]);
    const int r = lane & 15, g = lane >> 4;
    const int qi = r;
    const long qrow = q_base + (long)min(qi, d.nq - 1) * d.q_axis_stride;
    long krow[NKB], krow_v[NKB];
#pragma unroll
    for (int kb = 0; kb < NKB; ++kb) {
        krow[kb] = (kv_base + (long)min(kb * 16 + r, d.nk - 1) * d.kv_axis_stride) * d.ldk;
        krow_v[kb] = (kv_base + (long)min(kb * 16 + r, d.nk - 1) * d.kv_axis_stride) * d.ldv;
    }
    constexpr int CH = 4, VP = 40;
    __shared__ unsigned short vsm[4][CH][NKB * 16][VP];
    const int wv = threadIdx.x >> 6;
    uint4 kf[1][CH][NKB], qf[1][CH];
    ashort4 vt[1][CH][2][NKB];
    auto load_chunk = [&](int buf, int h0) {
#pragma unroll
        for (int t = 0; t < CH; ++t) {
            const int h = min(h0 + t, d.n_head - 1);
            qf[buf][t] = *(const uint4*)(qp + qrow * d.ldq + h * 32 + g * 8);
#pragma unroll
            for (int kb = 0; kb < NKB; ++kb) {
                kf[buf][t][kb] = *(const uint4*)(kp + krow[kb] + h * 32 + g * 8);
                *(uint4*)&vsm[wv][t][kb * 16 + r][g * 8] = *(const uint4*)(vp + krow_v[kb] + h * 32 + g * 8);
            }
        }
        __builtin_amdgcn_wave_barrier();
#pragma unroll
        for (int t = 0; t < CH; ++t)
#pragma unroll
            for (int kb = 0; kb < NKB; ++kb)
#pragma unroll
                for (int b = 0; b < 2; ++b)
#pragma unroll
                    for (int e = 0; e < 4; ++e) vt[buf][t][b][kb][e] = (short)vsm[wv][t][kb * 16 + 4 * g + e][b * 16 + r];
        __builtin_amdgcn_wave_barrier();
    };
    const int jmax_p = d.causal ? min(klen, (r & 1) + 1 + (d.nk - d.nq)) : klen;
    auto compute_chunk = [&](int buf, int h0) {
        f32x4 sp[NKB];
        auto gather = [&](auto T) {
            constexpr int t = decltype(T)::value;
#pragma unroll
            for (int kb = 0; kb < NKB; ++kb) {
                const f32x4 stt = attn_mfma_qk<HT>(kf[buf][t][kb], qf[buf][t]);
#pragma unroll
                for (int e = 0; e < 4; ++e) sp[kb][e] = row_shr_f<2 * t>(sp[kb][e], stt[e]);
            }
        };
        gather(std::integral_constant<int, 0>{});
        gather(std::integral_constant<int, 1>{});
        gather(std::integral_constant<int, 2>{});
        gather(std::integral_constant<int, 3>{});
        float mx = -INFINITY;
#pragma unroll
        for (int kb = 0; kb < NKB; ++kb)
#pragma unroll
            for (int e = 0; e < 4; ++e) {
                sp[kb][e] = (kb * 16 + 4 * g + e < jmax_p) ? sp[kb][e] * d.scale : -INFINITY;
                mx = fmaxf(mx, sp[kb][e]);
            }
        mx = fmaxf(mx, __shfl_xor(mx, 16));
        mx = fmaxf(mx, __shfl_xor(mx, 32));
        float den = 0.f;
        ashort4 phi_p[NKB], plo_p[NKB];
#pragma unroll
        for (int kb = 0; kb < NKB; ++kb)
#pragma unroll
            for (int e = 0; e < 4; ++e) {
                const float p = (kb * 16 + 4 * g + e < jmax_p) ? expf(sp[kb][e] - mx) : 0.f;
                den += p;
                short ph, pl;
                attn_p_split<HT>(p, ph, pl);
                phi_p[kb][e] = ph;
                plo_p[kb][e] = pl;
            }
        den += __shfl_xor(den, 16);
        den += __shfl_xor(den, 32);
        const float inv_p = 1.0f / den;
        auto finish = [&](auto T) {
            constexpr int t = decltype(T)::value;
            const int h = h0 + t;
            if (h >= d.n_head) return;
            ashort4 phi[NKB], plo[NKB];
#pragma unroll
            for (int kb = 0; kb < NKB; ++kb) {
                phi[kb] = row_shl_s4<2 * t>(phi_p[kb]);
                plo[kb] = row_shl_s4<2 * t>(plo_p[kb]);
            }
            const float inv = row_shl_f<2 * t>(inv_p);
            f32x4 o[2];
#pragma unroll
            for (int b = 0; b < 2; ++b) {
                o[b] = f32x4{0.f, 0.f, 0.f, 0.f};
#pragma unroll
                for (int kb = 0; kb < NKB; ++kb) {
                    o[b] = attn_mfma_pv<HT>(vt[buf][t][b][kb], phi[kb], o[b]);
                    o[b] = attn_mfma_pv<HT>(vt[buf][t][b][kb], plo[kb], o[b]);
                }
            }
            f32x4 v0, v1;
#pragma unroll
            for (int e = 0; e < 4; ++e) {
                const auto sw = __builtin_amdgcn_permlane16_swap(__float_as_uint(o[0][e]), __float_as_uint(o[1][e]), false, false);
                v0[e] = __uint_as_float(sw[0]) * inv;
                v1[e] = __uint_as_float(sw[1]) * inv;
            }
            if (qi < d.nq) {
                const int col = h * 32 + 16 * (g & 1) + 8 * (g >> 1);
                store8(op + (o_base + (long)qi * o_step) * d.ldo + col, v0, v1);
            }
        };
        finish(std::integral_constant<int, 0>{});
        finish(std::integral_constant<int, 1>{});
        finish(std::integral_constant<int, 2>{});
        finish(std::integral_constant<int, 3>{});
// ... 838 lines not shown
```

### mage_amd/csrc/runtime.hip

```cpp
#include <mutex>
#include "common.h"
#include <string.h>
#include <stdlib.h>

static thread_local char g_err[512] = "";
static void* g_zero[MAGE_MAX_DEVICES] = {nullptr};
static int* g_flag[MAGE_MAX_DEVICES] = {nullptr};

void mage_set_error(const char* fmt, ...) {
    va_list ap;
    va_start(ap, fmt);
    vsnprintf(g_err, sizeof(g_err), fmt, ap);
    va_end(ap);
}

int mage_device_index() {
    int dev = 0;
    if (hipGetDevice(&dev) != hipSuccess || dev < 0 || dev >= MAGE_MAX_DEVICES) return -1;
    return dev;
}

const void* mage_zero_page() {
    const int dev = mage_device_index();
    return dev < 0 ? nullptr : g_zero[dev];
}

int* mage_error_word() {
    const int dev = mage_device_index();
    return dev < 0 ? nullptr : g_flag[dev];
}

static MageOptions g_opt;
static std::once_flag g_opt_once;
struct OptField { const char* name; int MageOptions::*field; int hi; };
static const OptField g_opt_fields[] = {
    {"gemm_no_4w", &MageOptions::gemm_no_4w, 1}, {"gemm_no_4h", &MageOptions::gemm_no_4h, 1}, {"gemm_4h_plain", &MageOptions::gemm_4h_plain, 1},
    {"gemm4_train_forms", &MageOptions::gemm4_train_forms, 1}, {"gemm_no_8phase", &MageOptions::gemm_no_8phase, 1}, {"gemm_no_taps8", &MageOptions::gemm_no_taps8, 1},
    {"gemm_no_narrow", &MageOptions::gemm_no_narrow, 1}, {"gemm_no_narrow_few", &MageOptions::gemm_no_narrow_few, 1},
    {"gemm_no_small", &MageOptions::gemm_no_small, 1}, {"gemm_small_m", &MageOptions::gemm_small_m, 1 << 20},
    {"gemm_stagger_groups", &MageOptions::gemm_stagger_groups, 64},
    {"gemm_stagger_percent", &MageOptions::gemm_stagger_percent, 400}, {"gemm_stagger_forced", &MageOptions::gemm_stagger_forced, 1},
    {"gemm4_stagger_groups", &MageOptions::gemm4_stagger_groups, 64}, {"gemm4_stagger_percent", &MageOptions::gemm4_stagger_percent, 400},
    {"attn_no_mfma", &MageOptions::attn_no_mfma, 1}, {"attn_no_fewq", &MageOptions::attn_no_fewq, 1}, {"vq_no_mfma", &MageOptions::vq_no_mfma, 1},
    {"conv_no_tile", &MageOptions::conv_no_tile, 1},
};
static int env_flag(const char* name) {
    const char* e = getenv(name);
    return (e && *e && strcmp(e, "0") != 0) ? 1 : 0;
}
const MageOptions& mage_options() {
    std::call_once(g_opt_once, [] {
        MageOptions o = {};
        o.gemm_no_4w = env_flag("MAGE_GEMM_NO_4W");
        o.gemm_no_4h = env_flag("MAGE_GEMM_NO_4H");
        o.gemm_4h_plain = env_flag("MAGE_GEMM_4H_PLAIN");
        o.gemm4_train_forms = env_flag("MAGE_GEMM4_TRAIN_FORMS");
        o.gemm_no_8phase = env_flag("MAGE_GEMM_NO_8PHASE");
        o.gemm_no_taps8 = env_flag("MAGE_GEMM_NO_TAPS8");
        o.gemm_no_narrow = env_flag("MAGE_GEMM_NO_NARROW");
        o.gemm_no_narrow_few = env_flag("MAGE_GEMM_NO_NARROW_FEW");
        o.gemm_no_small = env_flag("MAGE_GEMM_NO_SMALL");
        o.gemm_small_m = getenv("MAGE_GEMM_SMALL_M") ? atoi(getenv("MAGE_GEMM_SMALL_M")) : 1024;
        o.gemm_stagger_groups = 8;
        o.gemm_stagger_percent = 60;
        if (const char* e = getenv("MAGE_GEMM_STAGGER")) {
            o.gemm_stagger_forced = 1;
            if (sscanf(e, "%d,%d", &o.gemm_stagger_groups, &o.gemm_stagger_percent) < 2) o.gemm_stagger_percent = 60;
        }
        o.gemm4_stagger_groups = 8;
        o.gemm4_stagger_percent = 100;
        if (const char* e = getenv("MAGE_GEMM4_STAGGER")) {
            if (sscanf(e, "%d,%d", &o.gemm4_stagger_groups, &o.gemm4_stagger_percent) < 2) o.gemm4_stagger_percent = 100;
        }
        o.attn_no_mfma = env_flag("MAGE_ATTN_NO_MFMA");
        o.attn_no_fewq = env_flag("MAGE_ATTN_NO_FEWQ");
        o.vq_no_mfma = env_flag("MAGE_VQ_NO_MFMA");
        o.conv_no_tile = env_flag("MAGE_CONV_NO_TILE");
        for (const OptField& f : g_opt_fields) {
            int& v = o.*(f.field);
            v = v < 0 ? 0 : v > f.hi ? f.hi : v;
        }
        g_opt = o;
    });
    return g_opt;
}
extern "C" int mage_set_option(const char* name, int32_t value) {
    MAGE_CHECK_ARG(name != nullptr, "mage_set_option: null name");
    (void)mage_options();
    for (const OptField& f : g_opt_fields)
        if (strcmp(f.name, name) == 0) {
            MAGE_CHECK_ARG(value >= 0 && value <= f.hi, "mage_set_option: value %d out of range for '%s' (0..%d)", (int)value, name, f.hi);
            g_opt.*(f.field) = value;
            return MAGE_OK;
        }
    mage_set_error("mage_set_option: unknown option '%s'", name);
    return MAGE_EINVAL;
}
extern "C" int mage_get_option(const char* name, int32_t* value) {
    MAGE_CHECK_ARG(name != nullptr && value != nullptr, "mage_get_option: null argument");
    const MageOptions& o = mage_options();
    for (const OptField& f : g_opt_fields)
        if (strcmp(f.name, name) == 0) {
            *value = o.*(f.field);
            return MAGE_OK;
        }
    mage_set_error("mage_get_option: unknown option '%s'", name);
    return MAGE_EINVAL;
}

int mage_gemm_cu_count() {
    static int n_cu_dev[MAGE_MAX_DEVICES] = {0};
    const int dev = mage_device_index();
    if (dev < 0) return 256;
    if (!n_cu_dev[dev]) {
        hipDeviceProp_t p;
        n_cu_dev[dev] = (hipGetDeviceProperties(&p, dev) == hipSuccess && p.multiProcessorCount >= 8) ? (p.multiProcessorCount & ~7) : 256;
    }
    return n_cu_dev[dev];
}

extern "C" int mage_abi_version(void) { return MAGE_ABI_VERSION; }

extern "C" const char* mage_last_error(void) { return g_err; }

extern "C" int mage_init(int device) {
    if (device < 0 || device >= MAGE_MAX_DEVICES) {
        mage_set_error("mage_init: device %d out of range", device);
        return MAGE_EINVAL;
    }
    if (g_zero[device]) return MAGE_OK;
    hipDeviceProp_t p;
    hipError_t e = hipGetDeviceProperties(&p, device);
    if (e == hipSuccess && strncmp(p.gcnArchName, "gfx950", 6) != 0) {
        mage_set_error("mage_init: device %d is %s; this library is built for gfx950 (MI355X) only", device, p.gcnArchName);
        return MAGE_EUNSUPPORTED;
    }
    int prev = -1;
    void* zero = nullptr;
    int* flag = nullptr;
    if (e == hipSuccess) e = hipGetDevice(&prev);
    if (e == hipSuccess) e = hipSetDevice(device);
    if (e == hipSuccess) e = hipMalloc(&zero, 16384);
    if (e == hipSuccess) e = hipMemset(zero, 0, 16384);
    if (e == hipSuccess) e = hipMalloc((void**)&flag, 16);
    if (e == hipSuccess) e = hipMemset(flag, 0, 16);
    if (e == hipSuccess) e = hipDeviceSynchronize();
    if (prev >= 0 && prev != device) (void)hipSetDevice(prev);
    if (e != hipSuccess) {
        if (zero) (void)hipFree(zero);
        if (flag) (void)hipFree(flag);
        mage_set_error("mage_init: %s", hipGetErrorString(e));
        return MAGE_EHIP;
    }
    g_flag[device] = flag;
    g_zero[device] = zero;
    return MAGE_OK;
}

extern "C" int mage_check_device_errors(void* stream) {
    int* flag = mage_error_word();
    MAGE_CHECK_ARG(flag != nullptr, "mage_check_device_errors: mage_init() has not been called on the current device");
    int host[4] = {0, 0, 0, 0};
    hipError_t e = hipMemcpyAsync(host, flag, 16, hipMemcpyDeviceToHost, (hipStream_t)stream);
    if (e == hipSuccess) e = hipStreamSynchronize((hipStream_t)stream);
    if (e != hipSuccess) {
        mage_set_error("mage_check_device_errors: %s", hipGetErrorString(e));
        return MAGE_EHIP;
    }
    if (host[0] == 0) return MAGE_OK;
    (void)hipMemsetAsync(flag, 0, 16, (hipStream_t)stream);
    const char* what = host[0] == MAGE_DEVERR_EMBEDDING_ID ? "mage_embedding: index out of range"
                       : host[0] == MAGE_DEVERR_CE_TARGET ? "mage_cross_entropy: target out of range"
                       : host[0] == MAGE_DEVERR_TOKEN_ID ? "mage_token_logprob: token out of range"
                                                          : "device-side argument error";
    mage_set_error("%s (value %d, valid range [0, %d))", what, host[1], host[2]);
    return MAGE_EINVAL;
}
```

### mage_amd/modules/mage_model.py

```python
from __future__ import annotations

import ctypes
import gc
import math
from collections import OrderedDict
from math import exp
from typing import Dict, Optional, Tuple

import torch
from torch import nn

from .. import config, ops
from ..utils.util import default, instantiate_from_config, zero_module
from .vqvae_model import VectorQuantizedVAE, _Derived, _conv_w, _no_torch_forward, weights_frozen

__all__ = ["QuickGELU", "AxialAttentionBlock", "TransformerBlock", "MAEncoder", "TransformerTextEncoder", "BasicBlock",
           "ADAIN2D", "FlatAxialDecoder", "PIDControl", "MAGE"]

F32 = torch.float32
BF16 = torch.bfloat16
F16 = torch.float16
HALF_TYPES = (BF16, F16)


# ... 378 lines not shown
            wp[:self.out_channels] = w
            bp = torch.zeros(n8, device=w.device)
            bp[:self.out_channels] = self.out[2].bias.float()
            _pack_linear(d, "out", wp, bp)
        d["tpos"] = self.T_positional_embedding.float().reshape(self.frames_length, self.model_channels).contiguous()
        for i, blk in enumerate(self.blocks):
            _pack_block(d, f"b{i}", blk)
            for ln, lin in (("ln_1", "in_proj"), ("ln_2", "c_fc")):
                w, g, bt = d[f"b{i}.{lin}.f32"], d[f"b{i}.{ln}.w"], d[f"b{i}.{ln}.b"]
                wq = (w * g[None, :]).to(BF16)
                d[f"b{i}.{lin}.lnw"] = wq
                d[f"b{i}.{lin}.lns"] = wq.float().sum(dim=1).contiguous()
                d[f"b{i}.{lin}.lnc"] = ((w.double() * bt.double()[None, :]).sum(1) + d[f"b{i}.{lin}.b"].double()).float().contiguous()
        return d

    def _fold(self, dt, B: int, hw: int) -> bool:
        return (dt in HALF_TYPES and (B * hw) % 256 == 0 and self.model_channels % 256 == 0 and config.get().ln_fold)

    def _stream_bf16(self) -> bool:
        return getattr(self, "stream_bf16", True) and config.get().stream_16bit

    def _ln_linear(self, d, p, lin, xn, xb, ln, y, *, M, N, **kw):
        Cc, name = self.model_channels, f"{p}.{lin}"
        if ln is None:
            return ops.gemm(xn, _wdt(d, name, self.compute_dtype), y, M=M, N=N, K=Cc, lda=Cc, ldy=N, bias=d[name + ".b"], **kw)
        lnw, lns = self._ln_fold_w(d, p, lin, xb.dtype)
        return ops.gemm(xb, lnw, y, M=M, N=N, K=Cc, lda=Cc, ldy=N, bias=d[name + ".lnc"], ln_colsum=lns, **ln, **kw)

    @staticmethod
    def _ln_fold_w(d, p, lin, dt):
        if dt == BF16:
            return d[f"{p}.{lin}.lnw"], d[f"{p}.{lin}.lns"]
        kw_, ks_ = f"{p}.{lin}.lnw.f16", f"{p}.{lin}.lns.f16"
        if kw_ not in d:
            ln = "ln_1" if lin == "in_proj" else "ln_2"
            wq = (d[f"{p}.{lin}.f32"] * d[f"{p}.{ln}.w"][None, :]).to(F16)
            d[kw_], d[ks_] = wq, wq.float().sum(dim=1).contiguous()
        return d[kw_], d[ks_]

    def _stats_inline(self, xb, M: int) -> bool:
        Cc = self.model_channels
        return all(ops.gemm_is_small(xb, M, n, Cc) for n in (Cc, 2 * Cc, 3 * Cc, 4 * Cc))

    @torch.no_grad()
    def _run(self, motion: torch.Tensor, imgs: torch.Tensor, *, B: int, hh: int, ww: int) -> torch.Tensor:
        L = self.frames_length
        run = self._pass_split if self._split_on() else self._pass
        return run(motion, imgs, B=B, hh=hh, ww=ww, p0=0, P=L, nf=L - 1, cache=None)

    def _inc_begin(self, B: int, hh: int, ww: int) -> dict:
        return {"B": B, "hh": hh, "ww": ww, "kv": {}, "p": 0}

    @torch.no_grad()
    def _inc_step(self, st: dict, motion: Optional[torch.Tensor], imgs: torch.Tensor) -> torch.Tensor:
        p0 = st["p"]
        P = 2 if motion is not None else 1
        assert self.use_cids and (p0 == 0) == (motion is not None) and p0 + P <= self.frames_length
        run = self._pass_split if self._split_on() else self._pass
        logits = run(motion, imgs, B=st["B"], hh=st["hh"], ww=st["ww"], p0=p0, P=P, nf=1, cache=st["kv"])
        st["p"] = p0 + P
        return logits

    def _axial_geo(self, axis: int, B: int, hh: int, ww: int, P: int, p0: int = 0, *, cached: bool = False,
                   q_cached: bool = False) -> dict:
        hw, H = hh * ww, self.model_channels // 32
        if axis == 1:
            return dict(n_seq=B * P * ww, inner=ww, nq=hh, nk=hh, q_outer_stride=hw, q_axis_stride=ww, causal=False,
                        kv_outer_stride=hw, kv_axis_stride=ww, n_head=H)
        if axis == 2:
            return dict(n_seq=B * P * hh, inner=1, nq=ww, nk=ww, q_outer_stride=ww, q_axis_stride=1, causal=False,
                        kv_outer_stride=ww, kv_axis_stride=1, n_head=H)
        kvo = (self.frames_length if cached else P) * hw
        geo = dict(n_seq=B * hw, inner=hw, nq=P, nk=p0 + P, q_outer_stride=kvo if q_cached else P * hw, q_axis_stride=hw, causal=True,
                   kv_outer_stride=kvo, kv_axis_stride=hw, n_head=H)
        if q_cached:
            geo.update(o_outer_stride=P * hw, o_axis_stride=hw)
        return geo

    def _embed(self, d, x, motion, imgs, *, B: int, hw: int, P: int, nf: int, tp: torch.Tensor, sk: int = 0) -> None:
        dt, Cc = self.compute_dtype, self.model_channels
        if motion is not None:
            if sk and self._taps_ok(B * hw):
                self._lin_s(ops.split(motion, sk), d, "context_linear", x, M=B * hw, N=Cc, K=self.context_channels, out_w=hw,
                            y_img_stride=P * hw, rowadd=tp, rowadd_div=hw, rowadd_mod=P)
            else:
                _linear(motion, d, "context_linear", x, dt, M=B * hw, N=Cc, K=self.context_channels, out_w=hw, y_img_stride=P * hw,
                        rowadd=tp, rowadd_div=hw, rowadd_mod=P)
        off = (P - nf) * hw
        if isinstance(imgs, FrameTokens):
            imgs.fill(x, n_img=B * nf, per_clip=nf, P=P, y_off=off, tp=tp)
        elif sk and imgs.dtype != F32:
            self._lin_s(imgs, d, "in_linear", x, M=B * nf * hw, N=Cc, K=self.in_channels, out_w=nf * hw, y_img_stride=P * hw, y_off=off,
                        rowadd=tp, rowadd_div=hw, rowadd_mod=P)
        else:
            _linear(imgs, d, "in_linear", x, dt, M=B * nf * hw, N=Cc, K=self.in_channels, out_w=nf * hw, y_img_stride=P * hw, y_off=off,
                    rowadd=tp, rowadd_div=hw, rowadd_mod=P)

    def _head(self, d, xa, *, B: int, hw: int, P: int, nf: int, split: bool = False) -> torch.Tensor:
        dt, Cc, rows = self.compute_dtype, self.model_channels, B * nf * hw
        if not self.use_cids:
            y = ops.groupnorm_silu(xa, d["gn.w"], d["gn.b"], torch.empty(rows, Cc, device=xa.device, dtype=dt), n_samples=B,
                                   rows_per_sample=nf * hw, sample_stride_rows=P * hw, row_off=(P - nf) * hw, groups=32, eps=self.out[0].eps)
            n8 = d["out.f32"].shape[0]
            return _linear(y, d, "out", torch.empty(rows, n8, device=xa.device, dtype=F32), dt, M=rows, N=n8, K=Cc)
        logits = torch.empty(rows, self.out_channels, device=xa.device, dtype=F32)
        if split:
            return self._lin_s(xa, d, "out", logits, M=rows, N=self.out_channels, K=Cc, out_w=nf * hw, a_img_stride=P * hw, a_off=(P - nf) * hw)
        return _linear(xa, d, "out", logits, dt, M=rows, N=self.out_channels, K=Cc, out_w=nf * hw, a_img_stride=P * hw, a_off=(P - nf) * hw)

    def _pass(self, motion, imgs, *, B: int, hh: int, ww: int, p0: int, P: int, nf: int, cache: Optional[dict]) -> torch.Tensor:
        d = self._derived.get(self._build)
        dt, Cc, L = self.compute_dtype, self.model_channels, self.frames_length
        dev = (imgs.tokens if isinstance(imgs, FrameTokens) else imgs).device
        hw = hh * ww
        M = B * P * hw
        fold = self._fold(dt, B, hw)
        sb = fold and self._stream_bf16()
        xb = part = stats = None
        if fold:
            xb = torch.empty(M, Cc, device=dev, dtype=dt)
            part = torch.empty(Cc // 64, M, 2, device=dev, dtype=F32)
            stats = torch.empty(M, 2, device=dev, dtype=F32)
        inl = fold and self._stats_inline(xb, M)
        ln = None if not fold else dict(ln_part=part, ln_eps=1e-5) if inl else dict(ln_stats=stats)
        ln0 = dict(ln_stats=stats) if sb else None
        x = xb if sb else torch.empty(M, Cc, device=dev, dtype=F32)
        res = dict(residual=x, ldr=Cc)
        if fold:
            res["ln_part"] = part
            if not sb:
                res.update(y2=xb, ldy2=Cc)
        self._embed(d, x, motion, imgs, B=B, hw=hw, P=P, nf=nf, tp=d["tpos"][p0:])
        if sb:
            ops.row_stats(xb, 1e-5, stats)
        xn = torch.empty(M, Cc, device=dev, dtype=dt)
        qkv = torch.empty(M, 3 * Cc, device=dev, dtype=dt)
        ao = torch.empty(M, Cc, device=dev, dtype=dt)
        hdn = torch.empty(M, 4 * Cc, device=dev, dtype=dt)
        geo = [self._axial_geo(a, B, hh, ww, P, p0, cached=cache is not None, q_cached=cache is not None) for a in range(3)]
        for i in range(self.layers):
            p = f"b{i}"
            ln1 = ln if i else ln0
            if ln1 is None:
                ops.layernorm(x, d[p + ".ln_1.w"], d[p + ".ln_1.b"], xn, 1e-5)
            if i % 3 == 0 and cache is not None:
                if p0 == 0:
                    cache[i] = torch.empty(B * L * hw, 3 * Cc, device=dev, dtype=dt)
                kv = cache[i]
                self._ln_linear(d, p, "in_proj", xn, xb, ln1, kv, M=M, N=3 * Cc, out_w=P * hw, y_img_stride=L * hw, y_off=p0 * hw)
                q = kv[p0 * hw:]
            else:
                q = kv = qkv
                self._ln_linear(d, p, "in_proj", xn, xb, ln1, qkv, M=M, N=3 * Cc)
            ops.attention(q, kv[:, Cc:], kv[:, 2 * Cc:], ao, ldq=3 * Cc, ldk=3 * Cc, ldv=3 * Cc, ldo=Cc, **geo[i % 3])
            _linear(ao, d, p + ".out_proj", x, dt, M=M, N=Cc, K=Cc, **res)
            if fold and not inl:
                ops.ln_stats(part, Cc, 1e-5, stats)
            if ln is None:
                ops.layernorm(x, d[p + ".ln_2.w"], d[p + ".ln_2.b"], xn, 1e-5)
            self._ln_linear(d, p, "c_fc", xn, xb, ln, hdn, M=M, N=4 * Cc, act=ops.ACT_QUICKGELU)
            if i < self.layers - 1:
                _linear(hdn, d, p + ".c_proj", x, dt, M=M, N=Cc, K=4 * Cc, **res)
                if fold and not inl:
                    ops.ln_stats(part, Cc, 1e-5, stats)
            else:
                if self.use_cids and dt != F32:
                    xa = xn
                else:
                    xa = torch.empty(M, Cc, device=dev, dtype=F32) if sb else x
                _linear(hdn, d, p + ".c_proj", xa, dt, M=M, N=Cc, K=4 * Cc, residual=x, ldr=Cc)
        return self._head(d, xa, B=B, hw=hw, P=P, nf=nf)

    def _split_on(self) -> bool:
        return bool(self.split_kind) and self.compute_dtype == F32 and self.model_channels % 64 == 0

    def _warm_split(self) -> None:
        if not self._split_on():
            return
        d = self._derived.get(self._build)
        names = ["in_linear", "context_linear"] + (["out"] if self.use_cids else [])
        for i in range(self.layers):
            names += [f"b{i}.in_proj", f"b{i}.out_proj", f"b{i}.c_fc", f"b{i}.c_proj"]
        for n in names:
            _wsplit(d, n, self.split_kind)

    def _attn_split(self) -> bool:
        return (self.split_kind == ops.F16X3 and self.frames_length <= 32 and (self.model_channels // 32) % 2 == 0
                and config.get().attn_split)

    def _taps_ok(self, rows: int) -> bool:
        return self.model_channels % 256 == 0 and rows % 256 == 0 and self.in_channels % 64 == 0 and self.context_channels % 64 == 0

    def _lin_s(self, a, d, name, y, *, M, N, K, lo=0, hi=None, **kw):
        sk = self.split_kind
        w, b = _wsplit(d, name, sk), d.get(name + ".b")
        if hi is not None or lo:
            w, b = w[lo:hi], (None if b is None else b[lo:hi])
        y_split = kw.pop("y_split", False)
        return ops.gemm(a, w, y, M=M, N=N, K=K, lda=kw.pop("lda", 2 * K), ldy=kw.pop("ldy", 2 * N if y_split else N), bias=b,
                        split_kind=sk, y_split=y_split, **kw)

    def _pass_split(self, motion, imgs, *, B: int, hh: int, ww: int, p0: int, P: int, nf: int, cache: Optional[dict]) -> torch.Tensor:
        d = self._derived.get(self._build)
        sk, Cc, L = self.split_kind, self.model_channels, self.frames_length
        dev = (imgs.tokens if isinstance(imgs, FrameTokens) else imgs).device
        hw = hh * ww
        M = B * P * hw
        x = torch.empty(M, Cc, device=dev, dtype=F32)
        self._embed(d, x, motion, imgs, B=B, hw=hw, P=P, nf=nf, tp=d["tpos"][p0:], sk=sk)
        xn = ops.split_empty(M, Cc, sk, dev)
        qs = self._attn_split()
        m_ = 2 if qs else 1
        qkv = ops.split_empty(M, 3 * Cc, sk, dev) if qs else torch.empty(M, 3 * Cc, device=dev, dtype=F32)
        ao = ops.split_empty(M, Cc, sk, dev)
        hdn = ops.split_empty(M, 4 * Cc, sk, dev)
        geo = [self._axial_geo(a, B, hh, ww, P, p0, cached=cache is not None) for a in range(3)]
        for i in range(self.layers):
            p = f"b{i}"
            ops.layernorm(x, d[p + ".ln_1.w"], d[p + ".ln_1.b"], xn, 1e-5, split_kind=sk)
            if i % 3 == 0 and cache is not None:
                if p0 == 0:
                    cache[i] = ops.split_empty(B * L * hw, 2 * Cc, sk, dev) if qs else torch.empty(B * L * hw, 2 * Cc, device=dev, dtype=F32)
                kv = cache[i]
                q = qkv.view(-1)[:M * m_ * Cc].view(M, m_ * Cc)
                self._lin_s(xn, d, p + ".in_proj", q, M=M, N=Cc, K=Cc, lo=0, hi=Cc, ldy=m_ * Cc, y_split=qs)
                self._lin_s(xn, d, p + ".in_proj", kv, M=M, N=2 * Cc, K=Cc, lo=Cc, hi=3 * Cc, ldy=m_ * 2 * Cc, out_w=P * hw,
                            y_img_stride=L * hw, y_off=p0 * hw, y_split=qs)
                k, v, ldq, ldkv = kv, kv[:, m_ * Cc:], m_ * Cc, m_ * 2 * Cc
            else:
                self._lin_s(xn, d, p + ".in_proj", qkv, M=M, N=3 * Cc, K=Cc, y_split=qs)
                q, k, v, ldq, ldkv = qkv, qkv[:, m_ * Cc:], qkv[:, m_ * 2 * Cc:], m_ * 3 * Cc, m_ * 3 * Cc
            ops.attention(q, k, v, ao, ldq=ldq, ldk=ldkv, ldv=ldkv, ldo=2 * Cc, out_split=sk, split_kind=sk if qs else 0, **geo[i % 3])
            self._lin_s(ao, d, p + ".out_proj", x, M=M, N=Cc, K=Cc, residual=x, ldr=Cc)
            ops.layernorm(x, d[p + ".ln_2.w"], d[p + ".ln_2.b"], xn, 1e-5, split_kind=sk)
            self._lin_s(xn, d, p + ".c_fc", hdn, M=M, N=4 * Cc, K=Cc, act=ops.ACT_QUICKGELU, y_split=True)
            if i == self.layers - 1 and self.use_cids:
                self._lin_s(hdn, d, p + ".c_proj", xn, M=M, N=Cc, K=4 * Cc, residual=x, ldr=Cc, y_split=True)
            else:
                self._lin_s(hdn, d, p + ".c_proj", x, M=M, N=Cc, K=4 * Cc, residual=x, ldr=Cc)
        return self._head(d, xn if self.use_cids else x, B=B, hw=hw, P=P, nf=nf, split=True)

    def forward(self, motion: torch.Tensor, imgs: torch.Tensor) -> torch.Tensor:
        _need_gpu(motion, "FlatAxialDecoder")
        B, hh, ww, _ = motion.shape
        dt = self.compute_dtype
        m = motion.reshape(B * hh * ww, -1).to(dt).contiguous()
        im = imgs.reshape(-1, imgs.shape[-1]).to(dt).contiguous()
        out = self._run(m, im, B=B, hh=hh, ww=ww)
        return out.view(B, self.frames_length - 1, hh, ww, -1)[..., :self.out_channels]


class PIDControl:

    def __init__(self):
        self.I_k1 = 0.0
        self.W_k1 = 0.0
        self.e_k1 = 0.0

    def _Kp_fun(self, Err, scale=1):
        return 1.0 / (1.0 + float(scale) * exp(Err))

    def pid(self, exp_KL, KL_loss, Kp=0.01, Ki=-0.0001, Kd=0.0):
        error_k = exp_KL - KL_loss
        Pk = Kp * self._Kp_fun(error_k)
        Ik = self.I_k1 + Ki * error_k
        if self.W_k1 < 0 and self.W_k1 >= 1:
            Ik = self.I_k1
        Wk = Pk + Ik
        self.W_k1, self.I_k1, self.e_k1 = Wk, Ik, error_k
        return min(max(Wk, 0.0), 1.0), error_k


def disabled_train(self, mode=True):
    return self


class MAGE(nn.Module):
    def __init__(self, first_stage_config, text_encoder_config, ma_config, generate_decoder_config, codebook_size: int,
                 frames_length: int, image_resolution: int, vision_width: int, dropout: float = 0.1, use_cids=False,
                 randomness=False, alpha=0., beta=1., v_kl=0., auto_beta=False):
        super().__init__()
        self.instantiate_first_stage(first_stage_config)
        self.frames_length, self.image_resolution, self.vision_width = frames_length, image_resolution, vision_width
        self.dropout, self.use_cids, self.auto_beta = dropout, use_cids, auto_beta
        self.text_encoder = instantiate_from_config(text_encoder_config)
        self.ma_encoder = instantiate_from_config(ma_config, {"dropout": dropout})
        if hasattr(self.ma_encoder, "mage_plus"):
            self.ma_encoder.mage_plus = not use_cids
        self.generate_model = instantiate_from_config(
            generate_decoder_config, {"use_cids": use_cids, "dropout": dropout, "context_channels": ma_config["params"]["d_model"]})
        self.codebook_size = codebook_size
        if use_cids:
            self.visual_token_embedding = nn.Embedding(codebook_size, vision_width)
        else:
            self.visual_token_embedding = nn.Linear(self.first_stage_model.embed_dim, vision_width)
        self.conv = nn.Sequential(nn.Conv2d(vision_width, vision_width, kernel_size=3, stride=1, padding=1, bias=False))
        scale = vision_width ** -0.5
        self.speed_embedding = nn.Parameter(scale * torch.randn(1, vision_width))
        self.H_positional_embedding = nn.Parameter(scale * torch.randn(1, image_resolution, 1, vision_width))
        self.W_positional_embedding = nn.Parameter(scale * torch.randn(1, 1, image_resolution, vision_width))
        self.randomness = randomness
        if randomness:
            dm = ma_config["params"]["d_model"]
            self.conv3d = nn.Sequential(*[BasicBlock(vision_width, vision_width if i < 3 else dm, stride=1, stride_t=2,
                                                     downsample=True) for i in range(4)])
            self.conv_mu2 = nn.Conv2d(vision_width, 64, 3, 1, 1)
            self.conv_var2 = nn.Conv2d(vision_width, 64, 3, 1, 1)
            self.conv_d2 = nn.Conv2d(64, vision_width, kernel_size=3, stride=1, padding=1, bias=False)
# ... 714 lines not shown
```

### mage_amd/ops.py

```python
from __future__ import annotations

import ctypes as C
from typing import Optional

import torch

from . import _lib
from ._lib import ACT_GELU_ERF, ACT_NONE, ACT_QUICKGELU, ACT_QUICKGELU_GRAD, ACT_RELU, ACT_TANH, BF16, BF16X3, F16, F16X3, F32, AttnDesc, GemmDesc

__all__ = ["gemm", "layernorm", "attention", "embedding", "table_conv", "split_rows", "vq_prepare", "vq_nearest", "argmax", "cross_entropy",
           "conv_in", "conv_out", "convt_fold_tanh", "row_affine", "groupnorm_silu", "groupnorm_act", "reparam_kl", "mse", "check_device_errors", "graph_events_supported", "transpose", "row_sum", "sum_partials", "layernorm_bwd", "dropout_add_layernorm", "act", "act_bwd", "cross_entropy_bwd", "embedding_bwd", "group_rowsum", "attention_bwd", "dropout", "adam", "bn_train_stats", "bn_apply", "bn_backward", "convt_unfold_tanh_bwd", "maxpool2", "upsample2", "relu", "cast", "adain", "add_scaled_rowvec",
           "token_logprob", "clip_scores", "split", "split_empty", "split_dtype", "PROFILE", "F32", "BF16", "F16", "BF16X3", "F16X3", "ACT_NONE", "ACT_RELU", "ACT_QUICKGELU", "ACT_GELU_ERF", "ACT_TANH", "tdtype", "code"]


def code(t: torch.Tensor) -> int:
    if t.dtype == torch.float32:
        return F32
    if t.dtype == torch.bfloat16:
        return BF16
    if t.dtype == torch.float16:
        return F16
    raise TypeError(f"unsupported dtype {t.dtype}")


# ... 7 lines not shown

def split_empty(rows: int, C_: int, kind: int, device, zero: bool = False) -> torch.Tensor:
    assert C_ % 64 == 0 and kind in (BF16X3, F16X3)
    f = torch.zeros if zero else torch.empty
    return f(rows, 2 * C_, device=device, dtype=split_dtype(kind))


def split(x: torch.Tensor, kind: int, out: Optional[torch.Tensor] = None) -> torch.Tensor:
    l, s = _dev(x)
    assert x.dtype == torch.float32 and x.dim() == 2 and x.stride(1) == 1
    rows, C_ = x.shape
    if out is None:
        out = split_empty(rows, C_, kind, x.device)
    assert out.dtype == split_dtype(kind) and out.is_contiguous() and out.shape[-1] == 2 * C_
    _lib.check(l.mage_split(x.data_ptr(), x.stride(0), out.data_ptr(), 2 * C_, rows, C_, kind, s), l)
    return out


def _dev(t: torch.Tensor):
    if not t.is_cuda:
        raise RuntimeError("mage_amd ops need tensors on a ROCm GPU (cuda device); there is no CPU fallback")
    idx = t.device.index or 0
    if idx != torch.cuda.current_device():
        raise RuntimeError(f"mage_amd ops: tensor on cuda:{idx} but the current device is cuda:{torch.cuda.current_device()}; "
                           f"wrap the call in torch.cuda.device({idx})")
    return _lib.lib(idx), torch.cuda.current_stream(t.device).cuda_stream


_GRAPH_EVENTS = {}


def graph_events_supported(device) -> bool:
    dev = torch.device(device)
    idx = dev.index if dev.index is not None else torch.cuda.current_device()
    if idx not in _GRAPH_EVENTS:
        ok = False
        import warnings
        try:
            with torch.cuda.device(idx), warnings.catch_warnings():
                warnings.simplefilter("ignore")
                x = torch.zeros(1 << 20, device=dev)
                torch.cuda.synchronize()
                g = torch.cuda.CUDAGraph()
                a = torch.cuda.Event(enable_timing=True, external=True)
                b = torch.cuda.Event(enable_timing=True, external=True)
                with torch.cuda.graph(g):
                    a.record()
                    x.add_(1.0)
                    b.record()
                for _ in range(2):
                    g.replay()
                    torch.cuda.synchronize()
                    ms = a.elapsed_time(b)
                ok = 0.0 < ms < 100.0
        except Exception:
            ok = False
        _GRAPH_EVENTS[idx] = ok
    return _GRAPH_EVENTS[idx]


def check_device_errors(device) -> None:
    dev = torch.device(device)
    idx = dev.index if dev.index is not None else torch.cuda.current_device()
    with torch.cuda.device(idx):
        l = _lib.lib(idx)
        _lib.check(l.mage_check_device_errors(torch.cuda.current_stream(idx).cuda_stream), l)


def _p(t: Optional[torch.Tensor]):
    return None if t is None else t.data_ptr()


def _kernel_name(l, d) -> str:
    buf = C.create_string_buffer(256)
    _lib.check(l.mage_gemm_kernel_name(C.byref(d), buf, len(buf)), l)
    return buf.value.decode()


class _Profile:

    def __init__(self):
        self.enabled = False
        self.records = []
        self.only = None
        self.external = False
        self.acc = {}

    def reset(self, enabled: bool = False, only=None):
        self.enabled, self.records, self.only = enabled, [], (set(only) if only is not None else None)
        self.acc = {}

    def clear(self):
        self.records, self.acc = [], {}

    def mode_key(self):
        if not self.enabled:
            return "off"
        return "all" if self.only is None else tuple(sorted(self.only))

    def wants(self, key: str) -> bool:
        return self.enabled and (self.only is None or key in self.only)

    def begin(self):
        e = torch.cuda.Event(enable_timing=True, external=True) if self.external else torch.cuda.Event(enable_timing=True)
        e.record()
        return e

    def end(self, key: str, start, flops: float = 0.0, nbytes: float = 0.0):
        e = torch.cuda.Event(enable_timing=True, external=True) if self.external else torch.cuda.Event(enable_timing=True)
        e.record()
        self.records.append((key, start, e, flops, nbytes))

    def capture_begin(self):
        saved = (self.records, self.external)
        self.records, self.external = [], True
        return saved

    def capture_end(self, saved):
        recs = self.records
        self.records, self.external = saved
        return recs

    def _add(self, out, recs):
        for key, s, e, fl, nb in recs:
            d = out.setdefault(key, {"ms": 0.0, "calls": 0, "flops": 0.0, "bytes": 0.0})
            d["ms"] += s.elapsed_time(e)
            d["calls"] += 1
            d["flops"] += fl
            d["bytes"] += nb

    def absorb(self, recs):
        if self.enabled and recs:
            self._add(self.acc, recs)

    def summary(self):
        torch.cuda.synchronize()
        out = {k: dict(v) for k, v in self.acc.items()}
        self._add(out, self.records)
        return out


PROFILE = _Profile()


def gemm(a: torch.Tensor, w: torch.Tensor, y: torch.Tensor, *, M: int, N: int, K: int, lda: int, ldy: int,
         out_h: int = 1, out_w: Optional[int] = None, in_h: Optional[int] = None, in_w: Optional[int] = None,
         a_img_stride: Optional[int] = None, a_off: int = 0, taps_h: int = 1, taps_w: int = 1, cin: Optional[int] = None,
         stride: int = 1, dy0: int = 0, dx0: int = 0, dys: int = 1, dxs: int = 1,
         y_img_stride: Optional[int] = None, y_mul_y: Optional[int] = None, y_mul_x: int = 1, y_off: int = 0,
         bias=None, scale=None, shift=None, act: int = ACT_NONE, rowadd=None, rowadd_div: int = 1, rowadd_mod: int = 1,
         residual=None, ldr: int = 0, post_relu: bool = False, ldw: int = 0, n_split: int = 1, a_split_stride: int = 0,
         w_split_stride: int = 0, y_split_stride: int = 0, y2=None, ldy2: int = 0, ln_part=None, ln_stats=None,
         ln_colsum=None, res_half: bool = False, a_half: bool = False, split_kind: int = 0, y_split: bool = False,
         ln_eps: float = 0.0, head_w=None, head_phases: int = 0, a_relu: bool = False) -> torch.Tensor:
    l, s = _dev(a)
    if split_kind and a_relu:
        raise ValueError("ops.gemm: split-precision operands (split_kind) do not take a_relu")
    if split_kind:
        unsupported = dict(scale=scale, shift=shift, y2=y2, ln_part=ln_part, ln_stats=ln_stats, ln_colsum=ln_colsum, head_w=head_w)
        bad = [k for k, v_ in unsupported.items() if v_ is not None]
        bad += [k for k, v_ in dict(post_relu=post_relu, res_half=res_half, a_half=a_half).items() if v_]
        bad += [k for k, v_ in dict(n_split=n_split).items() if v_ not in (0, 1)]
        bad += [k for k, v_ in dict(a_split_stride=a_split_stride, w_split_stride=w_split_stride, y_split_stride=y_split_stride, ldy2=ldy2,
                                    stride=stride - 1, dy0=dy0, dx0=dx0, dys=dys - 1, dxs=dxs - 1).items() if v_]
        if ln_eps:
            bad.append("ln_eps")
        if bad:
            raise ValueError(f"ops.gemm: split-precision operands (split_kind) do not take {', '.join(bad)}")
        if residual is not None and residual.dtype != torch.float32:
            raise ValueError(f"ops.gemm: the split-precision x + Linear(.) form adds an fp32 residual, got {residual.dtype}")
        return _gemm_split(l, s, a, w, y, M=M, N=N, K=K, lda=lda, ldy=ldy, out_h=out_h, out_w=out_w, in_h=in_h, in_w=in_w,
                           a_img_stride=a_img_stride, a_off=a_off, taps_h=taps_h, taps_w=taps_w, cin=cin, y_img_stride=y_img_stride,
                           y_mul_y=y_mul_y, y_mul_x=y_mul_x, y_off=y_off, bias=bias, act=act, rowadd=rowadd, rowadd_div=rowadd_div,
                           rowadd_mod=rowadd_mod, residual=residual, ldr=ldr, ldw=ldw, split_kind=split_kind, y_split=y_split)
    out_w = M if out_w is None else out_w
    in_h = out_h if in_h is None else in_h
    in_w = out_w if in_w is None else in_w
    d = GemmDesc()
    d.dtype, d.M, d.N, d.K = code(a), M, N, K
    assert w.dtype == a.dtype, (w.dtype, a.dtype)
    d.A, d.W, d.Y = a.data_ptr(), w.data_ptr(), y.data_ptr()
    d.lda, d.ldy, d.y_dtype = lda, ldy, code(y)
    d.out_h, d.out_w, d.in_h, d.in_w = out_h, out_w, in_h, in_w
    d.a_img_stride = in_h * in_w if a_img_stride is None else a_img_stride
    d.a_off = a_off
    d.taps_h, d.taps_w, d.cin, d.stride = taps_h, taps_w, (K // (taps_h * taps_w) if cin is None else cin), stride
    d.dy0, d.dx0, d.dys, d.dxs = dy0, dx0, dys, dxs
    d.y_img_stride = out_h * out_w if y_img_stride is None else y_img_stride
    d.y_mul_y = out_w if y_mul_y is None else y_mul_y
    d.y_mul_x, d.y_off = y_mul_x, y_off
    d.bias, d.scale, d.shift = _p(bias), _p(scale), _p(shift)
    d.act = act
    d.rowadd, d.rowadd_div, d.rowadd_mod = _p(rowadd), rowadd_div, rowadd_mod
    d.residual, d.ldr, d.res_dtype = _p(residual), ldr, (code(residual) if residual is not None else 0)
    d.post_relu = int(post_relu)
    d.ldw, d.n_split = ldw, n_split
    d.a_split_stride, d.w_split_stride, d.y_split_stride = a_split_stride, w_split_stride, y_split_stride
    d.y2, d.ldy2, d.ln_part, d.ln_stats, d.ln_colsum = _p(y2), ldy2, _p(ln_part), _p(ln_stats), _p(ln_colsum)
    d.ln_eps = float(ln_eps)
    if ln_part is not None:
        assert ln_part.dtype == torch.float32 and ln_part.dim() == 3 and ln_part.shape[2] == 2 and ln_part.is_contiguous(), tuple(ln_part.shape)
        d.ln_part_rows = ln_part.shape[1]
    if head_w is not None:
        assert head_w.dtype == torch.bfloat16 and head_w.is_contiguous() and tuple(head_w.shape) == (16, N // (head_phases or 1)) \
            and y.dtype == torch.float32, (head_w.dtype, tuple(head_w.shape), y.dtype)
    d.head_w = _p(head_w)
    d.head_phases = head_phases if head_w is not None else 0
    d.res_half = int(res_half)
    d.a_half = int(a_half)
    d.a_relu = int(a_relu)
    if PROFILE.enabled:
        key = _kernel_name(l, d)
        if PROFILE.wants(key):
            ev = PROFILE.begin()
            _lib.check(l.mage_gemm(C.byref(d), s), l)
            es, ys = a.element_size(), y.element_size()
            nb = float(M) * K * es + float(N) * K * es + float(M) * N * ys
            if key == "conv3x3_c64_kernel":
                nb = float(M) * 64 * es * (0.25 if a_half else 1.0) + float(N) * K * es + float(M) * N * ys
            if residual is not None:
                nb += float(M) * N * residual.element_size()
            if y2 is not None:
                nb += float(M) * N * 2
            if ln_part is not None:
                nb += float(M) * (N // 64) * 8
            fl = 2.0 * M * N * K
            if head_w is not None:
                nb += float(M) * 16 * 4 * (head_phases or 1) - float(M) * N * ys
                fl += 2.0 * M * N * 16
            PROFILE.end(key, ev, fl, nb)
            return y
    _lib.check(l.mage_gemm(C.byref(d), s), l)
    return y


def gemm_is_small(a: torch.Tensor, M: int, N: int, K: int) -> bool:
    l, _ = _dev(a)
    r = l.mage_gemm_is_small(M, N, K)
    if r < 0:
        _lib.check(r, l)
    return r == 1


def _gemm_split(l, s, a, w, y, *, M, N, K, lda, ldy, out_h, out_w, in_h, in_w, a_img_stride, a_off, taps_h, taps_w, cin, y_img_stride, y_mul_y,
                y_mul_x, y_off, bias, act, rowadd, rowadd_div, rowadd_mod, residual, ldr, ldw, split_kind, y_split):
    sd = split_dtype(split_kind)
    assert a.dtype == sd and w.dtype == sd and (y.dtype == sd if y_split else y.dtype == torch.float32), (a.dtype, w.dtype, y.dtype)
    out_w = M if out_w is None else out_w
    in_h = out_h if in_h is None else in_h
    in_w = out_w if in_w is None else in_w
    d = GemmDesc()
    d.dtype, d.M, d.N, d.K = split_kind, M, N, K
    d.A, d.W, d.Y = a.data_ptr(), w.data_ptr(), y.data_ptr()
    d.lda, d.ldy, d.y_dtype = lda, ldy, (split_kind if y_split else F32)
    d.out_h, d.out_w, d.in_h, d.in_w = out_h, out_w, in_h, in_w
    d.a_img_stride = in_h * in_w if a_img_stride is None else a_img_stride
    d.a_off = a_off
    d.taps_h, d.taps_w, d.cin, d.stride = taps_h, taps_w, (K // (taps_h * taps_w) if cin is None else cin), 1
    d.dy0, d.dx0, d.dys, d.dxs = 0, 0, 1, 1
    d.y_img_stride = out_h * out_w if y_img_stride is None else y_img_stride
    d.y_mul_y = out_w if y_mul_y is None else y_mul_y
    d.y_mul_x, d.y_off = y_mul_x, y_off
    d.bias, d.act = _p(bias), act
    d.rowadd, d.rowadd_div, d.rowadd_mod = _p(rowadd), rowadd_div, rowadd_mod
    d.residual, d.ldr, d.res_dtype = _p(residual), ldr, F32
    d.ldw, d.n_split = ldw, 1
    if PROFILE.enabled:
        key = _kernel_name(l, d)
        if PROFILE.wants(key):
            ev = PROFILE.begin()
            _lib.check(l.mage_gemm(C.byref(d), s), l)
            nb = 4.0 * M * K + 4.0 * N * K + float(M) * N * 4 * (2 if residual is not None else 1)
            PROFILE.end(key, ev, 2.0 * M * N * K, nb)
            return y
    _lib.check(l.mage_gemm(C.byref(d), s), l)
    return y


def row_stats(x: torch.Tensor, eps: float, stats: torch.Tensor) -> torch.Tensor:
    l, s = _dev(x)
    assert x.dtype in (torch.bfloat16, torch.float16) and x.dim() == 2 and x.stride(1) == 1 and stats.is_contiguous() and stats.numel() >= 2 * x.shape[0]
    ev = PROFILE.begin() if PROFILE.wants("layernorm") else None
    _lib.check(l.mage_row_stats(x.data_ptr(), code(x), x.shape[0], x.shape[1], x.stride(0), float(eps), stats.data_ptr(), s), l)
    if ev is not None:
        PROFILE.end("layernorm", ev, 0.0, float(x.numel()) * 2)
    return stats


def ln_stats(part: torch.Tensor, C_: int, eps: float, stats: torch.Tensor) -> torch.Tensor:
    l, s = _dev(part)
    n_slices, rows = part.shape[0], part.shape[1]
    assert part.dtype == torch.float32 and part.is_contiguous() and stats.is_contiguous() and stats.numel() >= 2 * rows
    if PROFILE.wants("ln_stats_kernel"):
        ev = PROFILE.begin()
        _lib.check(l.mage_ln_stats(part.data_ptr(), rows, n_slices, C_, eps, stats.data_ptr(), s), l)
        PROFILE.end("ln_stats_kernel", ev, 0.0)
        return stats
    _lib.check(l.mage_ln_stats(part.data_ptr(), rows, n_slices, C_, eps, stats.data_ptr(), s), l)
    return stats


def layernorm(x: torch.Tensor, gamma: torch.Tensor, beta: torch.Tensor, y: torch.Tensor, eps: float, split_kind: int = 0) -> torch.Tensor:
    l, s = _dev(x)
    assert x.dtype == torch.float32 and x.is_contiguous() and y.is_contiguous()
    Cc = x.shape[-1]
    assert not split_kind or (y.dtype == split_dtype(split_kind) and y.numel() == 2 * x.numel())
    ev = PROFILE.begin() if PROFILE.wants("layernorm") else None
    _lib.check(l.mage_layernorm(x.data_ptr(), gamma.data_ptr(), beta.data_ptr(), y.data_ptr(), split_kind or code(y),
                                x.numel() // Cc, Cc, float(eps), s), l)
    if ev is not None:
        PROFILE.end("layernorm", ev, 0.0, float(x.numel()) * (4 + y.element_size()))
    return y


def attention(q, k, v, out, *, ldq, ldk, ldv, ldo, n_seq, inner, nq, nk, n_head, q_outer_stride, q_axis_stride,
              kv_outer_stride, kv_axis_stride, causal=False, kv_len=None, kv_len_div=1, scale=None, out_split: int = 0,
              drop_p: float = 0.0, drop_seed: int = 0, split_kind: int = 0, o_outer_stride: int = 0, o_axis_stride: int = 0):
    l, s = _dev(q)
    d = AttnDesc()
    d.dtype = split_kind or code(q)
    d.q, d.k, d.v, d.out = q.data_ptr(), k.data_ptr(), v.data_ptr(), out.data_ptr()
    d.ldq, d.ldk, d.ldv, d.ldo = ldq, ldk, ldv, ldo
    d.n_seq, d.inner, d.nq, d.nk, d.n_head = n_seq, inner, nq, nk, n_head
    d.q_outer_stride, d.q_axis_stride = q_outer_stride, q_axis_stride
    d.kv_outer_stride, d.kv_axis_stride = kv_outer_stride, kv_axis_stride
    d.causal = int(causal)
    d.kv_len, d.kv_len_div = _p(kv_len), kv_len_div
    d.scale = float(32 ** -0.5 if scale is None else scale)
    d.out_split = out_split
    d.drop_p, d.drop_seed = float(drop_p), int(drop_seed) & (2 ** 64 - 1)
    d.o_outer_stride, d.o_axis_stride = o_outer_stride, o_axis_stride
    ev = PROFILE.begin() if PROFILE.wants("attention") else None
    _lib.check(l.mage_attention(C.byref(d), s), l)
    if ev is not None:
        es = q.element_size()
        PROFILE.end("attention", ev, 4.0 * n_seq * nq * nk * n_head * 32, float(n_seq) * n_head * 32 * es * (2 * nq + 2 * nk))
    return out


def embedding(ids: torch.Tensor, table: torch.Tensor, out: torch.Tensor, *, relu: bool = False, group: Optional[int] = None,
              group_stride: Optional[int] = None, off: int = 0, inner: int = 0, inner_stride: int = 0, split_kind: int = 0) -> torch.Tensor:
    l, s = _dev(table)
    assert ids.dtype == torch.int64 and ids.is_contiguous() and table.dtype == torch.float32 and table.is_contiguous()
    n = ids.numel()
    group = n if group is None else group
    group_stride = group if group_stride is None else group_stride
    _lib.check(l.mage_embedding(ids.data_ptr(), table.data_ptr(), out.data_ptr(), split_kind or code(out), n, table.shape[1],
                                table.shape[0], int(relu), group, group_stride, off, inner, inner_stride, s), l)
    return out


def table_conv(ids: torch.Tensor, table: torch.Tensor, y: torch.Tensor, *, n_img: int, H: int, W: int, taps: int = 3, pos=None, bias=None,
               relu: bool = False, rowadd=None, split_kind: int = 0,
               rowadd_div: int = 1, rowadd_mod: int = 1, ldy: Optional[int] = None, group: Optional[int] = None,
               y_group_stride: Optional[int] = None, y_off: int = 0) -> torch.Tensor:
    l, s = _dev(table)
    assert ids.dtype == torch.int64 and ids.is_contiguous() and ids.numel() == n_img * H * W
    assert table.dim() == 3 and table.shape[0] == taps * taps and table.is_contiguous()
    Cc = table.shape[2]
    group = n_img * H * W if group is None else group
    y_group_stride = group if y_group_stride is None else y_group_stride
    ev = PROFILE.begin() if PROFILE.wants("table_conv") else None
    _lib.check(l.mage_table_conv(ids.data_ptr(), n_img, H, W, taps, taps, table.data_ptr(), code(table), table.shape[1], Cc, _p(pos), _p(bias),
                                 int(relu), _p(rowadd), rowadd_div, rowadd_mod, y.data_ptr(), split_kind or code(y), Cc if ldy is None else ldy, group,
                                 y_group_stride, y_off, s), l)
    if ev is not None:
        PROFILE.end("table_conv", ev, 0.0, float(n_img) * H * W * Cc * (taps * taps * table.element_size() + 4))
    return y


def resblock_table(ids: torch.Tensor, table: torch.Tensor, codebook: torch.Tensor, w1: torch.Tensor, y: torch.Tensor, *, n_img: int, H: int, W: int,
                   bias3: torch.Tensor, b1: torch.Tensor, scale1=None, shift1=None, post_relu: bool = False, ldy: int, y_img_stride: int,
                   y_row_pitch: int, y_off: int = 0) -> torch.Tensor:
    l, s = _dev(table)
    Cc = table.shape[2]
    assert ids.dtype == torch.int64 and ids.is_contiguous() and ids.numel() == n_img * H * W
    assert table.dtype == torch.bfloat16 and table.dim() == 3 and table.shape[0] == 9 and table.is_contiguous()
    assert codebook.dtype == torch.float32 and codebook.is_contiguous() and tuple(codebook.shape) == (table.shape[1], Cc)
    assert w1.dtype == torch.bfloat16 and w1.is_contiguous() and tuple(w1.shape) == (Cc, Cc) and y.dtype == torch.bfloat16
    ev = PROFILE.begin() if PROFILE.wants("resblock_table") else None
    _lib.check(l.mage_resblock_table(ids.data_ptr(), n_img, H, W, table.data_ptr(), table.shape[1], Cc, bias3.data_ptr(), codebook.data_ptr(),
                                     w1.data_ptr(), b1.data_ptr(), _p(scale1), _p(shift1), int(post_relu), y.data_ptr(), ldy, y_img_stride,
                                     y_row_pitch, y_off, s), l)
    if ev is not None:
        npix = float(n_img) * H * W
        PROFILE.end("resblock_table", ev, 2.0 * npix * Cc * Cc, npix * (8 + 2 * Cc))
    return y


def resblock_rows(t: torch.Tensor, w1: torch.Tensor, residual: torch.Tensor, y: torch.Tensor, *, n_img: int, H: int, W: int, b1: torch.Tensor,
                  scale1=None, shift1=None, post_relu: bool = False, lda: int, ldr: int, ldy: int, img_stride: int, row_pitch: int,
                  off: int = 0) -> torch.Tensor:
    l, s = _dev(t)
    Cc = w1.shape[0]
    assert t.dtype == torch.bfloat16 and w1.dtype == torch.bfloat16 and residual.dtype == torch.bfloat16 and y.dtype == torch.bfloat16
    assert w1.is_contiguous() and tuple(w1.shape) == (Cc, Cc)
    ev = PROFILE.begin() if PROFILE.wants("resblock_rows") else None
    _lib.check(l.mage_resblock_rows(t.data_ptr(), lda, w1.data_ptr(), b1.data_ptr(), _p(scale1), _p(shift1), residual.data_ptr(), ldr,
                                    int(post_relu), y.data_ptr(), ldy, n_img, H, W, Cc, img_stride, row_pitch, off, s), l)
    if ev is not None:
        npix = float(n_img) * H * W
        PROFILE.end("resblock_rows", ev, 2.0 * npix * Cc * Cc, npix * 3 * 2 * Cc)
    return y


def vq_prepare(codebook: torch.Tensor):
    l, s = _dev(codebook)
    K, D = codebook.shape
    cbt = torch.empty(D, K, device=codebook.device, dtype=torch.float32)
    c2 = torch.empty(K, device=codebook.device, dtype=torch.float32)
    _lib.check(l.mage_vq_prepare(codebook.contiguous().data_ptr(), K, D, cbt.data_ptr(), c2.data_ptr(), s), l)
    return cbt, c2


def vq_nearest(z: torch.Tensor, cbt: torch.Tensor, c2: torch.Tensor, want_margin: bool = False):
    l, s = _dev(z)
    assert z.dtype == torch.float32 and z.is_contiguous()
    D, K = cbt.shape
    M = z.numel() // D
    idx = torch.empty(M, device=z.device, dtype=torch.int64)
    margin = torch.empty(M, device=z.device, dtype=torch.float32) if want_margin else None
    _lib.check(l.mage_vq_nearest(z.data_ptr(), cbt.data_ptr(), c2.data_ptr(), M, D, K, idx.data_ptr(), _p(margin), s), l)
    return (idx, margin) if want_margin else idx


def argmax(logits: torch.Tensor, out: torch.Tensor, *, rows: int, K: int, ld: Optional[int] = None, group: Optional[int] = None,
           in_group_stride: Optional[int] = None, in_off: int = 0, out_group_stride: Optional[int] = None, out_off: int = 0,
           margin=None) -> torch.Tensor:
    l, s = _dev(logits)
    assert logits.dtype == torch.float32 and out.dtype == torch.int64
    group = rows if group is None else group
    in_group_stride = group if in_group_stride is None else in_group_stride
    out_group_stride = group if out_group_stride is None else out_group_stride
    _lib.check(l.mage_argmax(logits.data_ptr(), rows, K, K if ld is None else ld, group, in_group_stride, in_off,
                             out.data_ptr(), out_group_stride, out_off, _p(margin), s), l)
    return out


def sample_tokens(logits: torch.Tensor, out: torch.Tensor, seeds: torch.Tensor, *, rows: int, K: int, temperature: float = 1.0,
                  top_k: int = 0, top_p: float = 1.0, pos_off: int = 0, ld: Optional[int] = None, group: Optional[int] = None,
                  in_group_stride: Optional[int] = None, in_off: int = 0, out_group_stride: Optional[int] = None,
                  out_off: int = 0) -> torch.Tensor:
    l, s = _dev(logits)
    assert logits.dtype == torch.float32 and out.dtype == torch.int64 and seeds.dtype == torch.int64 and seeds.is_contiguous()
    group = rows if group is None else group
    in_group_stride = group if in_group_stride is None else in_group_stride
    out_group_stride = group if out_group_stride is None else out_group_stride
    assert seeds.device == logits.device and seeds.numel() >= (rows + group - 1) // group
    _lib.check(l.mage_sample_tokens(logits.data_ptr(), rows, K, K if ld is None else ld, group, in_group_stride, in_off,
                                    out.data_ptr(), out_group_stride, out_off, seeds.data_ptr(), pos_off, float(temperature),
                                    int(top_k), float(top_p), s), l)
    return out


def token_logprob(logits: torch.Tensor, tokens: torch.Tensor, logprob: torch.Tensor, *, rows: int, K: int, ld: Optional[int] = None,
                  group: Optional[int] = None, in_group_stride: Optional[int] = None, in_off: int = 0,
                  tok_group_stride: Optional[int] = None, tok_off: int = 0) -> torch.Tensor:
    l, s = _dev(logits)
    assert logits.dtype == torch.float32 and tokens.dtype == torch.int64 and logprob.dtype == torch.float32
    assert tokens.device == logits.device and logprob.device == logits.device
    group = rows if group is None else group
    in_group_stride = group if in_group_stride is None else in_group_stride
    tok_group_stride = group if tok_group_stride is None else tok_group_stride
    last = ((rows - 1) // group) * tok_group_stride + (rows - 1) % group + tok_off
    assert tok_off >= 0 and last < tokens.numel() and last < logprob.numel()
    _lib.check(l.mage_token_logprob(logits.data_ptr(), rows, K, K if ld is None else ld, group, in_group_stride, in_off, tokens.data_ptr(),
                                    logprob.data_ptr(), tok_group_stride, tok_off, s), l)
    return logprob


def clip_scores(logprob: torch.Tensor, *, n_clips: int, n_cand: int = 1):
    l, s = _dev(logprob)
    assert logprob.dtype == torch.float32 and logprob.is_contiguous() and logprob.numel() % (n_clips * n_cand) == 0
    scores = torch.empty(n_clips, n_cand, device=logprob.device, dtype=torch.float32)
    best = torch.empty(n_clips, device=logprob.device, dtype=torch.int64) if n_cand > 1 else None
    _lib.check(l.mage_clip_scores(logprob.data_ptr(), n_clips, n_cand, logprob.numel() // (n_clips * n_cand), scores.data_ptr(), _p(best), s), l)
    return scores, best


def cross_entropy(logits: torch.Tensor, target: torch.Tensor) -> torch.Tensor:
    l, s = _dev(logits)
    assert logits.dtype == torch.float32 and logits.is_contiguous() and target.dtype == torch.int64
    K = logits.shape[-1]
    rows = logits.numel() // K
    row_loss = torch.empty(rows, device=logits.device, dtype=torch.float32)
    loss = torch.empty(1, device=logits.device, dtype=torch.float32)
    _lib.check(l.mage_cross_entropy(logits.data_ptr(), target.contiguous().data_ptr(), rows, K, row_loss.data_ptr(),
                                    loss.data_ptr(), s), l)
    return loss[0]

# ... 444 lines not shown
```

Measured before the change: 5740.

## Fuse 16-token attention into the out-projection GEMM with residual epilogue

Adds a persistent kernel that computes the short-sequence (16x16) attention per head inside the out_proj GEMM. The attention output goes into shared memory as the A operand and is never written to or read back from global memory. The projection weights are streamed one head at a time and the existing lean epilogue applies bias, residual and layernorm partials. It is used for the non-temporal attention layers during uncached bf16/f16 generation when the number of tiles fills the CUs. This removes one kernel launch and the round trip of the attention output, at the cost of a complex, heavily specialised kernel with strict shape preconditions.

```diff
diff --git a/__graft_entry__.py b/__graft_entry__.py
--- a/__graft_entry__.py
+++ b/__graft_entry__.py
@@ -12,6 +12,7 @@
     env.setdefault("HIPCC", "/opt/rocm/bin/hipcc")
     subprocess.run(["make", "-C", os.path.join(ROOT, "mage_amd", "csrc"), "-j4"], check=True, env=env)
     subprocess.run(["make", "-C", os.path.join(ROOT, "mage_amd", "csrc"), "check4"], check=True, env=env)
+    subprocess.run(["make", "-C", os.path.join(ROOT, "mage_amd", "csrc"), "check_attn_proj"], check=True, env=env)
     import mage_amd
     from mage_amd import _lib
     lib = _lib.load()
diff --git a/include/mage_hip.h b/include/mage_hip.h
--- a/include/mage_hip.h
+++ b/include/mage_hip.h
@@ -22,6 +22,7 @@
 int mage_set_option(const char* name, int32_t value);
 int mage_get_option(const char* name, int32_t* value);
 
+typedef struct mage_attn_desc mage_attn_desc;
 typedef struct mage_gemm_desc {
     int32_t dtype;
     int32_t M, N, K;
@@ -59,6 +60,7 @@
     int32_t head_phases;
     int32_t a_relu;
     int64_t ln_part_rows;
+    const mage_attn_desc* a_attn;
 } mage_gemm_desc;
 
 int mage_gemm(const mage_gemm_desc* desc, void* stream);
diff --git a/mage_amd/_lib.py b/mage_amd/_lib.py
--- a/mage_amd/_lib.py
+++ b/mage_amd/_lib.py
@@ -32,6 +32,7 @@
         ("a_split_stride", i64), ("w_split_stride", i64), ("y_split_stride", i64),
         ("y2", vp), ("ldy2", i32), ("res_half", i32), ("ln_part", vp), ("ln_stats", vp), ("ln_colsum", vp), ("a_half", i32), ("ln_eps", C.c_float),
         ("head_w", vp), ("head_phases", i32), ("a_relu", i32), ("ln_part_rows", i64),
+        ("a_attn", vp),
     ]
 
 
diff --git a/mage_amd/config.py b/mage_amd/config.py
--- a/mage_amd/config.py
+++ b/mage_amd/config.py
@@ -55,7 +55,7 @@
 
 LIB_OPTIONS = ("gemm_no_4w", "gemm_no_4h", "gemm_4h_plain", "gemm4_train_forms", "gemm_no_8phase", "gemm_no_taps8", "gemm_no_narrow", "gemm_no_narrow_few", "gemm_no_small",
                "gemm_small_m", "gemm_stagger_groups", "gemm_stagger_percent", "gemm_stagger_forced",
-               "gemm4_stagger_groups", "gemm4_stagger_percent", "attn_no_mfma", "attn_no_fewq", "vq_no_mfma", "conv_no_tile")
+               "gemm4_stagger_groups", "gemm4_stagger_percent", "attn_no_mfma", "attn_no_fewq", "attn_proj", "vq_no_mfma", "conv_no_tile")
 
 
 def _set(v) -> bool:
diff --git a/mage_amd/csrc/attn_proj.hip b/mage_amd/csrc/attn_proj.hip
--- /dev/null
+++ b/mage_amd/csrc/attn_proj.hip
@@ -0,0 +1,224 @@
+#include "attn_unit.h"
+#include "gemm_shared.h"
+
+int mage_attn_proj_try(const mage_gemm_desc* d, hipStream_t s);
+
+namespace {
+
+struct AttnProjArgs {
+    mage_gemm_desc d;
+    mage_attn_desc a;
+    const char* zero;
+    int ntiles;
+};
+
+#define MAGE_ATTN_PROJ_MIN_TILES 1
+constexpr int AP_VP = 40;
+constexpr int AP_IMG = 128 * 64;
+constexpr int AP_V0 = 2 * AP_IMG;
+constexpr int AP_STG0 = AP_V0 + 8 * 16 * AP_VP * 2;
+constexpr int AP_W0 = AP_STG0 + 8 * 4096;
+constexpr int AP_B0 = AP_W0 + 8 * 8192;
+constexpr int AP_LDS = AP_B0 + 8 * 4096;
+
+template <bool HF, int NW>
+__global__ __launch_bounds__(512, 2) void attn_proj_kernel(const AttnProjArgs g) {
+    typedef std::conditional_t<HF, f16_t, unsigned short> HT;
+    constexpr int MT = NW;
+    constexpr int NH = NW * 2;
+    constexpr int C = NH * 32;
+    const mage_gemm_desc& d = g.d;
+    const mage_attn_desc& a = g.a;
+    extern __shared__ __attribute__((aligned(16))) char smem[];
+    const int lane = threadIdx.x & 63;
+    const int wave = __builtin_amdgcn_readfirstlane(threadIdx.x >> 6);
+    const int r = lane & 15, gq = lane >> 4;
+    const int wm = wave / NW, wn = wave % NW;
+    const int n0 = wn * 64;
+
+    const int nwg8 = gridDim.x >> 3;
+    const int xcd = blockIdx.x & 7, li = blockIdx.x >> 3;
+    const int q8 = g.ntiles >> 3, r8 = g.ntiles & 7;
+    const int chunk0 = xcd < r8 ? xcd * (q8 + 1) : r8 * (q8 + 1) + (xcd - r8) * q8;
+    const int chunk1 = chunk0 + q8 + (xcd < r8 ? 1 : 0);
+    int c_tile = chunk0 + li;
+    if (c_tile >= chunk1) return;
+
+    const char* qp = (const char*)a.q;
+    const char* kp = (const char*)a.k;
+    const char* vp = (const char*)a.v;
+    const char* wp = (const char*)d.W;
+    const int jmax = a.nk;
+    auto seq_base = [&](int s) {
+        const int outer = s / a.inner;
+        return outer * a.q_outer_stride + (s - outer * a.inner);
+    };
+
+    uint4 q0, k0, vv0, q1, k1, vv1;
+    int ld_h = 0;
+    unsigned ld_row = (unsigned)(seq_base(c_tile * 8 + wave) + r * a.q_axis_stride), ld_row_next = ld_row;
+    auto request = [&](uint4& q, uint4& k, uint4& v) {
+        const unsigned col = (unsigned)(ld_h * 64 + gq * 16);
+        q = *(const uint4*)(qp + (ld_row * (unsigned)(2 * a.ldq) + col));
+        k = *(const uint4*)(kp + (ld_row * (unsigned)(2 * a.ldk) + col));
+        v = *(const uint4*)(vp + (ld_row * (unsigned)(2 * a.ldv) + col));
+        const bool wrap = ++ld_h == NH;
+        ld_h = wrap ? 0 : ld_h;
+        ld_row = wrap ? ld_row_next : ld_row;
+    };
+    u32x4 wf[2][4];
+    const unsigned wlane = (unsigned)(((n0 + r) * C + gq * 8) * 2);
+    auto request_w = [&](u32x4 (&wf)[4], int h) {
+        unsigned wl = wlane;
+        asm volatile("" : "+v"(wl));
+#pragma unroll
+        for (int nt = 0; nt < 4; ++nt) wf[nt] = *(const u32x4*)(wp + (wl + (unsigned)(nt * 16 * C * 2 + h * 64)));
+    };
+    request(q0, k0, vv0);
+    request(q1, k1, vv1);
+
+    unsigned short* vsm = (unsigned short*)(smem + AP_V0) + wave * 16 * AP_VP;
+    char* stg = smem + AP_STG0 + wave * 4096;
+    const int img_w = (wave * 16 + r) * 64 + (2 * (gq & 1) + (gq >> 1)) * 16;
+    const int img_r = (wm * MT * 16 + r) * 64 + gq * 16;
+    f32x4 acc[MT][4];
+
+    auto step = [&](uint4& q, uint4& k, uint4& v, auto PAR, int h) __attribute__((always_inline)) {
+        constexpr int par = decltype(PAR)::value;
+        __builtin_amdgcn_s_waitcnt(0xC07F);
+        ring_barrier();
+        const char* img = smem + par * AP_IMG + img_r;
+        constexpr int FB = MT / 4;
+        u32x4 xf[2][FB];
+#pragma unroll
+        for (int i = 0; i < FB; ++i) xf[0][i] = *(const u32x4*)(img + i * 1024);
+        auto batch = [&](auto I) __attribute__((always_inline)) {
+            constexpr int b = decltype(I)::value;
+            __builtin_amdgcn_sched_barrier(0);
+            if constexpr (b + 1 < 4) {
+#pragma unroll
+                for (int i = 0; i < FB; ++i) xf[(b + 1) & 1][i] = *(const u32x4*)(img + ((b + 1) * FB + i) * 1024);
+            }
+#pragma unroll
+            for (int i = 0; i < FB; ++i)
+#pragma unroll
+                for (int nt = 0; nt < 4; ++nt) acc[b * FB + i][nt] = mfma16x16x32<HT>(wf[par][nt], xf[b & 1][i], acc[b * FB + i][nt]);
+            __builtin_amdgcn_sched_barrier(0);
+        };
+        *(uint4*)(vsm + r * AP_VP + gq * 8) = v;
+        __builtin_amdgcn_wave_barrier();
+        const uint4 kf[1] = {k};
+        f32x4 o0, o1;
+        attn_mfma_unit<1, HT>(kf, q, jmax, a.scale, gq, [&](int, int b) {
+            ashort4 vt;
+#pragma unroll
+            for (int e = 0; e < 4; ++e) vt[e] = (short)vsm[(4 * gq + e) * AP_VP + b * 16 + r];
+            return vt;
+        }, o0, o1, batch);
+        __builtin_amdgcn_wave_barrier();
+        *(uint4*)(smem + (par ^ 1) * AP_IMG + img_w) =
+            uint4{pack16x2<HT>(o0[0], o0[1]), pack16x2<HT>(o0[2], o0[3]), pack16x2<HT>(o1[0], o1[1]), pack16x2<HT>(o1[2], o1[3])};
+        __builtin_amdgcn_sched_barrier(0);
+        request_w(wf[par], (h + 2) & (NH - 1));
+        __builtin_amdgcn_sched_barrier(0);
+        request(q, k, v);
+        __builtin_amdgcn_sched_barrier(0);
+    };
+    auto attention0 = [&](uint4& q, uint4& k, uint4& v) {
+        *(uint4*)(vsm + r * AP_VP + gq * 8) = v;
+        __builtin_amdgcn_wave_barrier();
+        const uint4 kf[1] = {k};
+        f32x4 o0, o1;
+        attn_mfma_unit<1, HT>(kf, q, jmax, a.scale, gq, [&](int, int b) {
+            ashort4 vt;
+#pragma unroll
+            for (int e = 0; e < 4; ++e) vt[e] = (short)vsm[(4 * gq + e) * AP_VP + b * 16 + r];
+            return vt;
+        }, o0, o1);
+        __builtin_amdgcn_wave_barrier();
+        *(uint4*)(smem + img_w) = uint4{pack16x2<HT>(o0[0], o0[1]), pack16x2<HT>(o0[2], o0[3]), pack16x2<HT>(o1[0], o1[1]), pack16x2<HT>(o1[2], o1[3])};
+        request(q, k, v);
+    };
+
+    char* w0 = smem + AP_W0 + wave * 8192 + lane * 16;
+    request_w(wf[0], 0);
+    request_w(wf[1], 1);
+#pragma unroll
+    for (int i = 0; i < 2; ++i)
+#pragma unroll
+        for (int nt = 0; nt < 4; ++nt) *(u32x4*)(w0 + (i * 4 + nt) * 1024) = wf[i][nt];
+    char* b0 = smem + AP_B0 + wave * 4096 + lane * 16;
+    {
+        const char* bp = d.bias ? (const char*)d.bias : (const char*)g.zero;
+#pragma unroll
+        for (int nt = 0; nt < 4; ++nt) *(f32x4*)(b0 + nt * 1024) = *(const f32x4*)(bp + (unsigned)((n0 + nt * 16 + gq * 4) * 4));
+    }
+    attention0(q0, k0, vv0);
+
+    for (; c_tile < chunk1; c_tile += nwg8) {
+        ld_row_next = (unsigned)(seq_base((c_tile + nwg8 < chunk1 ? c_tile + nwg8 : c_tile) * 8 + wave) + r * a.q_axis_stride);
+#pragma unroll
+        for (int mt = 0; mt < MT; ++mt)
+#pragma unroll
+            for (int nt = 0; nt < 4; ++nt) acc[mt][nt] = f32x4{0.f, 0.f, 0.f, 0.f};
+#pragma unroll
+        for (int i = 0; i < 2; ++i)
+#pragma unroll
+            for (int nt = 0; nt < 4; ++nt) wf[i][nt] = *(const u32x4*)(w0 + (i * 4 + nt) * 1024);
+        for (int h = 0; h < NH; h += 2) {
+            step(q1, k1, vv1, std::integral_constant<int, 0>{}, h);
+            step(q0, k0, vv0, std::integral_constant<int, 1>{}, h + 1);
+        }
+        f32x4 biasm[4];
+#pragma unroll
+        for (int nt = 0; nt < 4; ++nt) biasm[nt] = *(const f32x4*)(b0 + nt * 1024);
+        int tbase[MT];
+#pragma unroll
+        for (int mt = 0; mt < MT; ++mt) tbase[mt] = seq_base(c_tile * 8 + wm * MT + mt);
+        epilogue_lean<MAGE_ACT_NONE, HT, MT, false, LN_PRODUCE, 0, HT, true, true>(d, biasm, acc, 0, n0, lane, 1, stg, 0, nullptr, tbase,
+                                                                                      a.q_axis_stride);
+    }
+}
+
+template <bool HF>
+int launch(const mage_gemm_desc* d, hipStream_t s, int n_cu) {
+    AttnProjArgs g;
+    g.d = *d;
+    g.a = *d->a_attn;
+    g.d.a_attn = nullptr;
+    g.zero = (const char*)mage_zero_page();
+    g.ntiles = g.a.n_seq / 8;
+    const int grid = g.ntiles >= n_cu ? n_cu : ((g.ntiles + 7) & ~7);
+    if (d->N == 512) return mage_gemm_launch<attn_proj_kernel<HF, 8>>(grid, 512, AP_LDS, s, g);
+    return mage_gemm_launch<attn_proj_kernel<HF, 4>>(grid, 512, AP_LDS, s, g);
+}
+
+}
+
+int mage_attn_proj_try(const mage_gemm_desc* d, hipStream_t s) {
+    const mage_attn_desc* a = d->a_attn;
+    const int mode = mage_options().attn_proj;
+    if (!a || mode == 0 || mage_options().attn_no_mfma) return 0;
+    const bool h16 = d->dtype == MAGE_BF16 || d->dtype == MAGE_F16;
+    const bool attn_ok = h16 && a->dtype == d->dtype && a->nq == 16 && a->nk == 16 && !a->causal && !a->kv_len && a->drop_p == 0.f && a->out_split == 0 &&
+                         a->n_seq > 0 && a->n_seq % 8 == 0 && a->inner >= 1 &&
+                         a->kv_outer_stride == a->q_outer_stride && a->kv_axis_stride == a->q_axis_stride && a->q_axis_stride == a->inner &&
+                         a->q_outer_stride == 16 * a->inner && ((a->o_outer_stride == 0 && a->o_axis_stride == 0) ||
+                                                               (a->o_outer_stride == a->q_outer_stride && a->o_axis_stride == a->q_axis_stride)) &&
+                         (a->ldq | a->ldk | a->ldv) % 8 == 0 && a->ldq >= d->K && a->ldk >= d->K && a->ldv >= d->K &&
+                         (int64_t)a->n_seq * 16 * 2 * (a->ldq > a->ldk ? (a->ldq > a->ldv ? a->ldq : a->ldv) : (a->ldk > a->ldv ? a->ldk : a->ldv)) < (1LL << 32) &&
+                         (((uintptr_t)a->q | (uintptr_t)a->k | (uintptr_t)a->v) & 15) == 0 && a->q && a->k && a->v;
+    if (!attn_ok) return 0;
+    const bool gemm_ok = a->n_head * 32 == d->K && d->K == d->N && (d->N == 256 || d->N == 512) && (long)a->n_seq * 16 == d->M && a->ldo == d->lda &&
+                         d->lda == d->K && d->a_off == 0 &&
+                         d->taps_h == 1 && d->taps_w == 1 && d->stride == 1 && d->dy0 == 0 && d->dx0 == 0 && d->out_h == 1 && d->in_h == 1 &&
+                         d->out_w >= d->M && d->in_w == d->out_w && d->y_mul_x == 1 && d->y_off == 0 && d->n_split == 1 && d->act == MAGE_ACT_NONE &&
+                         !d->scale && !d->rowadd && !d->post_relu && !d->a_half && !d->a_relu && !d->head_w && !d->y2 && !d->ln_stats && !d->ln_colsum &&
+                         d->residual && d->res_dtype == d->dtype && d->y_dtype == d->dtype && d->ln_part && d->ldr % 8 == 0 && d->ldy % 8 == 0 &&
+                         d->ldr >= d->N && d->ldy >= d->N && (((uintptr_t)d->residual) & 15) == 0;
+    if (!gemm_ok) return 0;
+    const int n_cu = mage_gemm_cu_count();
+    if (mode == 1 && a->n_seq / 8 < MAGE_ATTN_PROJ_MIN_TILES * n_cu) return 0;
+    const int rc = d->dtype == MAGE_F16 ? launch<true>(d, s, n_cu) : launch<false>(d, s, n_cu);
+    return rc == MAGE_OK ? 1 : rc;
+}
diff --git a/mage_amd/csrc/attn_unit.h b/mage_amd/csrc/attn_unit.h
--- /dev/null
+++ b/mage_amd/csrc/attn_unit.h
@@ -0,0 +1,85 @@
+#pragma once
+#include <type_traits>
+#include "common.h"
+
+typedef __attribute__((ext_vector_type(8))) __bf16 abf16x8;
+typedef __attribute__((ext_vector_type(4))) short ashort4;
+typedef __attribute__((ext_vector_type(4))) _Float16 ahalf4;
+template <typename HT> __device__ __forceinline__ void attn_p_split(float p, short& hi, short& lo) {
+    if constexpr (std::is_same<HT, f16_t>::value) {
+        const _Float16 h = (_Float16)p;
+        hi = __builtin_bit_cast(short, h);
+        lo = __builtin_bit_cast(short, (_Float16)(p - (float)h));
+    } else {
+        const unsigned hb = __float_as_uint(p) & 0xffff0000u;
+        hi = (short)(hb >> 16);
+        lo = (short)(__float_as_uint(p - __uint_as_float(hb)) >> 16);
+    }
+}
+template <typename HT> __device__ __forceinline__ f32x4 attn_mfma_pv(const ashort4& vt, const ashort4& p, const f32x4& o) {
+    if constexpr (std::is_same<HT, f16_t>::value)
+        return __builtin_amdgcn_mfma_f32_16x16x16f16(__builtin_bit_cast(ahalf4, vt), __builtin_bit_cast(ahalf4, p), o, 0, 0, 0);
+    else
+        return __builtin_amdgcn_mfma_f32_16x16x16bf16_1k(vt, p, o, 0, 0, 0);
+}
+template <typename HT> __device__ __forceinline__ f32x4 attn_mfma_qk(const uint4& k, const uint4& q) {
+    return mfma16x16x32<HT>(__builtin_bit_cast(u32x4, k), __builtin_bit_cast(u32x4, q), f32x4{0.f, 0.f, 0.f, 0.f});
+}
+
+struct AttnNoHook {
+    template <typename I> __device__ __forceinline__ void operator()(I) const {}
+};
+template <int NKB, typename HT, typename VFrag, typename Hook = AttnNoHook>
+__device__ __forceinline__ void attn_mfma_unit(const uint4 (&kf)[NKB], const uint4& qf, int jmax, float scale, int g, VFrag&& vfrag,
+                                               f32x4& v0, f32x4& v1, Hook&& hook = Hook()) {
+    f32x4 st[NKB];
+    float mx = -INFINITY;
+#pragma unroll
+    for (int kb = 0; kb < NKB; ++kb) {
+        st[kb] = attn_mfma_qk<HT>(kf[kb], qf);
+#pragma unroll
+        for (int e = 0; e < 4; ++e) {
+            st[kb][e] = (kb * 16 + 4 * g + e < jmax) ? st[kb][e] * scale : -INFINITY;
+            mx = fmaxf(mx, st[kb][e]);
+        }
+    }
+    hook(std::integral_constant<int, 0>{});
+    mx = fmaxf(mx, __shfl_xor(mx, 16));
+    mx = fmaxf(mx, __shfl_xor(mx, 32));
+    hook(std::integral_constant<int, 1>{});
+    float den = 0.f;
+    ashort4 phi[NKB], plo[NKB];
+#pragma unroll
+    for (int kb = 0; kb < NKB; ++kb)
+#pragma unroll
+        for (int e = 0; e < 4; ++e) {
+            const float p = (kb * 16 + 4 * g + e < jmax) ? expf(st[kb][e] - mx) : 0.f;
+            den += p;
+            short ph, pl;
+            attn_p_split<HT>(p, ph, pl);
+            phi[kb][e] = ph;
+            plo[kb][e] = pl;
+        }
+    den += __shfl_xor(den, 16);
+    den += __shfl_xor(den, 32);
+    hook(std::integral_constant<int, 2>{});
+    f32x4 o[2];
+#pragma unroll
+    for (int b = 0; b < 2; ++b) {
+        o[b] = f32x4{0.f, 0.f, 0.f, 0.f};
+#pragma unroll
+        for (int kb = 0; kb < NKB; ++kb) {
+            const ashort4 vt = vfrag(kb, b);
+            o[b] = attn_mfma_pv<HT>(vt, phi[kb], o[b]);
+            o[b] = attn_mfma_pv<HT>(vt, plo[kb], o[b]);
+        }
+    }
+    hook(std::integral_constant<int, 3>{});
+    const float inv = 1.0f / den;
+#pragma unroll
+    for (int e = 0; e < 4; ++e) {
+        const auto sw = __builtin_amdgcn_permlane16_swap(__float_as_uint(o[0][e]), __float_as_uint(o[1][e]), false, false);
+        v0[e] = __uint_as_float(sw[0]) * inv;
+        v1[e] = __uint_as_float(sw[1]) * inv;
+    }
+}
diff --git a/mage_amd/csrc/common.h b/mage_amd/csrc/common.h
--- a/mage_amd/csrc/common.h
+++ b/mage_amd/csrc/common.h
@@ -32,6 +32,7 @@
     int gemm4_stagger_groups, gemm4_stagger_percent;
     int attn_no_mfma;
     int attn_no_fewq;
+    int attn_proj;
     int vq_no_mfma;
     int conv_no_tile;
 };
diff --git a/mage_amd/csrc/gemm.hip b/mage_amd/csrc/gemm.hip
--- a/mage_amd/csrc/gemm.hip
+++ b/mage_amd/csrc/gemm.hip
@@ -6,6 +6,7 @@
 #include "gemm_impl.h"
 
 int mage_gemm_f16(const mage_gemm_desc* d, hipStream_t s);
+int mage_attn_proj_try(const mage_gemm_desc* d, hipStream_t s);
 
 #ifdef MAGE_PROBE
 extern "C" int mage_debug_read_waves(void* dst, size_t bytes) {
@@ -85,6 +86,16 @@
     MAGE_CHECK_ARG(!d->a_relu || (d->dtype == MAGE_BF16 && !gather_ && !d->a_half && d->N <= 128 && d->n_split == 1 && !d->residual && !d->rowadd && !d->scale &&
                                   !d->post_relu && !d->y2 && !d->ln_part && !d->ln_stats && !d->ln_colsum && !d->head_w),
                    "mage_gemm: a_relu is a form of the bf16 plain GEMM with N <= 128 (epilogue act(acc + bias) only)");
+    if (d->a_attn) {
+        MAGE_CHECK_ARG(d->a_attn->out == d->A && d->a_attn->ldo == d->lda && d->a_attn->dtype == d->dtype && d->a_attn->out_split == 0,
+                       "mage_gemm: a_attn must describe the attention that writes A (out == A, ldo == lda, the GEMM's dtype)");
+        if (const int r = mage_attn_proj_try(d, s)) return r < 0 ? r : MAGE_OK;
+        if (!mage_gemm_plan) {
+            const int r = mage_attention(d->a_attn, stream);
+            if (r != MAGE_OK) return r;
+        }
+        dn.a_attn = nullptr;
+    }
     if (spl) {
         const bool tapsform = gather_ || d->rowadd;
         MAGE_CHECK_ARG(!d->head_w, "mage_gemm: head_w is a fusion of the bf16 padded-taps form");
diff --git a/mage_amd/csrc/gemm_shared.h b/mage_amd/csrc/gemm_shared.h
--- a/mage_amd/csrc/gemm_shared.h
+++ b/mage_amd/csrc/gemm_shared.h
@@ -26,10 +26,12 @@
 enum { LN_NONE = 0, LN_PRODUCE = 1, LN_CONSUME = 2, LN_DUAL = 3, LN_GELUBWD = 4, LN_HEAD = 5 };
 
 template <int ACT, typename OT, int MT, bool AFFINE = false, int LN = LN_NONE, int OSPL = 0,
-          typename HT = std::conditional_t<sizeof(OT) == 2, OT, unsigned short>, bool RESE = false>
+          typename HT = std::conditional_t<sizeof(OT) == 2, OT, unsigned short>, bool RESE = false, bool ROWMAP = false>
 __device__ __forceinline__ void epilogue_lean(const mage_gemm_desc& d, const f32x4 (&bias)[4], f32x4 (&acc)[MT][4], int m0, int n0,
-                                              int lane, int plane, char* stg, long ysplit, const LnConsume* lnc = nullptr) {
+                                              int lane, int plane, char* stg, long ysplit, const LnConsume* lnc = nullptr,
+                                              [[maybe_unused]] const int* tbase = nullptr, [[maybe_unused]] int tstride = 0) {
     constexpr bool F32 = sizeof(OT) == 4;
+    static_assert(!ROWMAP || (RESE && !AFFINE && !F32), "per-tile row bases: the 16-bit x + Linear(.) form on plain rows");
     static_assert((LN != LN_DUAL && LN != LN_GELUBWD) || std::is_same<HT, unsigned short>::value, "training forms: bf16 rows");
     static_assert(!RESE || (sizeof(OT) == 2 && OSPL == 0 && (LN == LN_NONE || LN == LN_PRODUCE)), "residual in the epilogue: 16-bit rows out");
     constexpr int RB = F32 ? 256 : 128;
@@ -59,7 +61,7 @@
     for (int i = 0; i < NST; ++i) MAGE_DASSERT(roff[i] >= 0 && roff[i] + 16 <= 4096);
     const bool simple_rows = d.out_h == 1 && d.out_w >= d.M;
     const bool affine_rows = AFFINE && d.out_h == 1 && d.y_mul_x == 1 && d.out_w % 256 == 0;
-    const bool interior = (simple_rows || affine_rows) && m0 + MT * 16 <= d.M && n0 + 64 <= d.N;
+    const bool interior = ROWMAP || ((simple_rows || affine_rows) && m0 + MT * 16 <= d.M && n0 + 64 <= d.N);
     const bool cv_ok = col < d.N;
     const long row_shift = (AFFINE && !simple_rows && affine_rows) ? (long)(m0 / d.out_w) * (d.y_img_stride - d.out_w) : 0;
     const int ldy = OSPL ? d.ldy >> 1 : d.ldy;
@@ -79,14 +81,16 @@
         for (int i = 0; i < 2; ++i) auxr[mt & 1][i] = *(const u32x4*)(ap + (long)(8 * i) * d.y_mul_x * d.ldy2);
     };
     if constexpr (LN == LN_GELUBWD) aux_request(0);
-    constexpr int RD = 3;
+    constexpr int RD = ROWMAP ? 2 : 3;
     [[maybe_unused]] u32x4 rland[RESE ? RD : 1][2];
     [[maybe_unused]] const HT* rbase = nullptr;
     [[maybe_unused]] auto res_request = [&](int t) {
 #pragma unroll
         for (int i = 0; i < 2; ++i) {
             const int m = min(m0 + t * 16 + (lane >> 3) + 8 * i, d.M - 1);
-            if constexpr (AFFINE) {
+            if constexpr (ROWMAP) {
+                rland[t % RD][i] = *(const u32x4*)(rbase + (long)(tbase[t] + ((lane >> 3) + 8 * i) * tstride) * d.ldr);
+            } else if constexpr (AFFINE) {
                 const int img = m / plane, rem = m - img * plane;
                 const int oy = rem / d.out_w, ox = rem - oy * d.out_w;
                 const long rrow = d.res_half ? (long)img * (plane >> 2) + (long)(oy >> 1) * (d.out_w >> 1) + (ox >> 1) : (long)m;
@@ -179,7 +183,7 @@
             s1 += __shfl_xor(s1, 32);
             s2 += __shfl_xor(s2, 32);
             if (grp == 0) {
-                const long row = (long)(m0 + mt * 16 + l15) * d.y_mul_x + d.y_off;
+                const long row = ROWMAP ? (long)(tbase[mt] + l15 * tstride) : (long)(m0 + mt * 16 + l15) * d.y_mul_x + d.y_off;
                 float* pp = d.ln_part + ((long)(n0 >> 6) * d.ln_part_rows + row) * 2;
                 *(float2*)pp = float2{s1, s2};
             }
@@ -190,7 +194,9 @@
     auto store = [&](int mt, const u32x4 (&o)[NST]) {
 #pragma unroll
         for (int i = 0; i < NST; ++i) {
-            if (interior) {
+            if constexpr (ROWMAP) {
+                __builtin_nontemporal_store(o[i], (u32x4*)((OT*)d.Y + (long)(tbase[mt] + (rr + RPI * i) * tstride) * ldy + col));
+            } else if (interior) {
 #ifdef MAGE_EPI_NO_STORE
                 asm volatile("" ::"v"(o[i]), "v"(yp));
 #else
diff --git a/mage_amd/csrc/norm_attn.hip b/mage_amd/csrc/norm_attn.hip
--- a/mage_amd/csrc/norm_attn.hip
+++ b/mage_amd/csrc/norm_attn.hip
@@ -2,6 +2,7 @@
 #include <type_traits>
 
 #include "common.h"
+#include "attn_unit.h"
 
 namespace {
 
@@ -161,29 +162,6 @@
     }
 }
 
-typedef __attribute__((ext_vector_type(8))) __bf16 abf16x8;
-typedef __attribute__((ext_vector_type(4))) short ashort4;
-typedef __attribute__((ext_vector_type(4))) _Float16 ahalf4;
-template <typename HT> __device__ __forceinline__ void attn_p_split(float p, short& hi, short& lo) {
-    if constexpr (std::is_same<HT, f16_t>::value) {
-        const _Float16 h = (_Float16)p;
-        hi = __builtin_bit_cast(short, h);
-        lo = __builtin_bit_cast(short, (_Float16)(p - (float)h));
-    } else {
-        const unsigned hb = __float_as_uint(p) & 0xffff0000u;
-        hi = (short)(hb >> 16);
-        lo = (short)(__float_as_uint(p - __uint_as_float(hb)) >> 16);
-    }
-}
-template <typename HT> __device__ __forceinline__ f32x4 attn_mfma_pv(const ashort4& vt, const ashort4& p, const f32x4& o) {
-    if constexpr (std::is_same<HT, f16_t>::value)
-        return __builtin_amdgcn_mfma_f32_16x16x16f16(__builtin_bit_cast(ahalf4, vt), __builtin_bit_cast(ahalf4, p), o, 0, 0, 0);
-    else
-        return __builtin_amdgcn_mfma_f32_16x16x16bf16_1k(vt, p, o, 0, 0, 0);
-}
-template <typename HT> __device__ __forceinline__ f32x4 attn_mfma_qk(const uint4& k, const uint4& q) {
-    return mfma16x16x32<HT>(__builtin_bit_cast(u32x4, k), __builtin_bit_cast(u32x4, q), f32x4{0.f, 0.f, 0.f, 0.f});
-}
 
 template <int NKB, int MAXH, typename HT = unsigned short>
 __global__ __launch_bounds__(256) void attention_mfma_kernel(const mage_attn_desc d) {
@@ -239,56 +217,14 @@
         for (int t = 0; t < MAXH; ++t) {
             const int h = wave + 4 * t;
             if (h >= d.n_head) break;
-            f32x4 st[NKB];
-            float mx = -INFINITY;
-#pragma unroll
-            for (int kb = 0; kb < NKB; ++kb) {
-                st[kb] = attn_mfma_qk<HT>(kf[t][kb], qf[t]);
-#pragma unroll
-                for (int e = 0; e < 4; ++e) {
-                    st[kb][e] = (kb * 16 + 4 * g + e < jmax) ? st[kb][e] * d.scale : -INFINITY;
-                    mx = fmaxf(mx, st[kb][e]);
-                }
-            }
-            mx = fmaxf(mx, __shfl_xor(mx, 16));
-            mx = fmaxf(mx, __shfl_xor(mx, 32));
-            float den = 0.f;
-            ashort4 phi[NKB], plo[NKB];
-#pragma unroll
-            for (int kb = 0; kb < NKB; ++kb)
-#pragma unroll
-                for (int e = 0; e < 4; ++e) {
-                    const float p = (kb * 16 + 4 * g + e < jmax) ? expf(st[kb][e] - mx) : 0.f;
-                    den += p;
-                    short ph, pl;
-                    attn_p_split<HT>(p, ph, pl);
-                    phi[kb][e] = ph;
-                    plo[kb][e] = pl;
-                }
-            den += __shfl_xor(den, 16);
-            den += __shfl_xor(den, 32);
-            f32x4 o[2];
-#pragma unroll
-            for (int b = 0; b < 2; ++b) {
-                o[b] = f32x4{0.f, 0.f, 0.f, 0.f};
-#pragma unroll
-                for (int kb = 0; kb < NKB; ++kb) {
-                    const unsigned short* vr = vs + (kb * 16 + 4 * g) * vpitch + h * 32 + b * 16 + r;
-                    ashort4 vt;
-#pragma unroll
-                    for (int e = 0; e < 4; ++e) vt[e] = (short)vr[e * vpitch];
-                    o[b] = attn_mfma_pv<HT>(vt, phi[kb], o[b]);
-                    o[b] = attn_mfma_pv<HT>(vt, plo[kb], o[b]);
-                }
-            }
-            const float inv = 1.0f / den;
             f32x4 v0, v1;
-#pragma unroll
-            for (int e = 0; e < 4; ++e) {
-                const auto sw = __builtin_amdgcn_permlane16_swap(__float_as_uint(o[0][e]), __float_as_uint(o[1][e]), false, false);
-                v0[e] = __uint_as_float(sw[0]) * inv;
-                v1[e] = __uint_as_float(sw[1]) * inv;
-            }
+            attn_mfma_unit<NKB, HT>(kf[t], qf[t], jmax, d.scale, g, [&](int kb, int b) {
+                const unsigned short* vr = vs + (kb * 16 + 4 * g) * vpitch + h * 32 + b * 16 + r;
+                ashort4 vt;
+#pragma unroll
+                for (int e = 0; e < 4; ++e) vt[e] = (short)vr[e * vpitch];
+                return vt;
+            }, v0, v1);
             if (qi < d.nq) {
                 const int col = h * 32 + 16 * (g & 1) + 8 * (g >> 1);
                 store8(op + (o_base + (long)qi * o_step) * d.ldo + col, v0, v1);
diff --git a/mage_amd/csrc/runtime.hip b/mage_amd/csrc/runtime.hip
--- a/mage_amd/csrc/runtime.hip
+++ b/mage_amd/csrc/runtime.hip
@@ -41,7 +41,7 @@
     {"gemm_stagger_groups", &MageOptions::gemm_stagger_groups, 64},
     {"gemm_stagger_percent", &MageOptions::gemm_stagger_percent, 400}, {"gemm_stagger_forced", &MageOptions::gemm_stagger_forced, 1},
     {"gemm4_stagger_groups", &MageOptions::gemm4_stagger_groups, 64}, {"gemm4_stagger_percent", &MageOptions::gemm4_stagger_percent, 400},
-    {"attn_no_mfma", &MageOptions::attn_no_mfma, 1}, {"attn_no_fewq", &MageOptions::attn_no_fewq, 1}, {"vq_no_mfma", &MageOptions::vq_no_mfma, 1},
+    {"attn_no_mfma", &MageOptions::attn_no_mfma, 1}, {"attn_no_fewq", &MageOptions::attn_no_fewq, 1}, {"attn_proj", &MageOptions::attn_proj, 2}, {"vq_no_mfma", &MageOptions::vq_no_mfma, 1},
     {"conv_no_tile", &MageOptions::conv_no_tile, 1},
 };
 static int env_flag(const char* name) {
@@ -74,6 +74,7 @@
         }
         o.attn_no_mfma = env_flag("MAGE_ATTN_NO_MFMA");
         o.attn_no_fewq = env_flag("MAGE_ATTN_NO_FEWQ");
+        o.attn_proj = getenv("MAGE_ATTN_PROJ") ? atoi(getenv("MAGE_ATTN_PROJ")) : 1;
         o.vq_no_mfma = env_flag("MAGE_VQ_NO_MFMA");
         o.conv_no_tile = env_flag("MAGE_CONV_NO_TILE");
         for (const OptField& f : g_opt_fields) {
diff --git a/mage_amd/modules/mage_model.py b/mage_amd/modules/mage_model.py
--- a/mage_amd/modules/mage_model.py
+++ b/mage_amd/modules/mage_model.py
@@ -554,8 +554,12 @@
             else:
                 q = kv = qkv
                 self._ln_linear(d, p, "in_proj", xn, xb, ln1, qkv, M=M, N=3 * Cc)
-            ops.attention(q, kv[:, Cc:], kv[:, 2 * Cc:], ao, ldq=3 * Cc, ldk=3 * Cc, ldv=3 * Cc, ldo=Cc, **geo[i % 3])
-            _linear(ao, d, p + ".out_proj", x, dt, M=M, N=Cc, K=Cc, **res)
+            if i % 3 != 0 and cache is None and dt != F32:
+                _linear(ao, d, p + ".out_proj", x, dt, M=M, N=Cc, K=Cc, **res,
+                        a_attn=dict(q=q, k=kv[:, Cc:], v=kv[:, 2 * Cc:], ldq=3 * Cc, ldk=3 * Cc, ldv=3 * Cc, **geo[i % 3]))
+            else:
+                ops.attention(q, kv[:, Cc:], kv[:, 2 * Cc:], ao, ldq=3 * Cc, ldk=3 * Cc, ldv=3 * Cc, ldo=Cc, **geo[i % 3])
+                _linear(ao, d, p + ".out_proj", x, dt, M=M, N=Cc, K=Cc, **res)
             if fold and not inl:
                 ops.ln_stats(part, Cc, 1e-5, stats)
             if ln is None:
diff --git a/mage_amd/ops.py b/mage_amd/ops.py
--- a/mage_amd/ops.py
+++ b/mage_amd/ops.py
@@ -183,8 +183,10 @@
          residual=None, ldr: int = 0, post_relu: bool = False, ldw: int = 0, n_split: int = 1, a_split_stride: int = 0,
          w_split_stride: int = 0, y_split_stride: int = 0, y2=None, ldy2: int = 0, ln_part=None, ln_stats=None,
          ln_colsum=None, res_half: bool = False, a_half: bool = False, split_kind: int = 0, y_split: bool = False,
-         ln_eps: float = 0.0, head_w=None, head_phases: int = 0, a_relu: bool = False) -> torch.Tensor:
+         ln_eps: float = 0.0, head_w=None, head_phases: int = 0, a_relu: bool = False, a_attn: Optional[dict] = None) -> torch.Tensor:
     l, s = _dev(a)
+    if split_kind and a_attn is not None:
+        raise ValueError("ops.gemm: split-precision operands (split_kind) do not take a_attn")
     if split_kind and a_relu:
         raise ValueError("ops.gemm: split-precision operands (split_kind) do not take a_relu")
     if split_kind:
@@ -240,6 +242,11 @@
     d.res_half = int(res_half)
     d.a_half = int(a_half)
     d.a_relu = int(a_relu)
+    ad = None
+    if a_attn is not None:
+        kw = dict(a_attn)
+        ad = _attn_desc(kw.pop("q"), kw.pop("k"), kw.pop("v"), a, ldo=lda, **kw)
+        d.a_attn = C.addressof(ad)
     if PROFILE.enabled:
         key = _kernel_name(l, d)
         if PROFILE.wants(key):
@@ -247,6 +254,8 @@
             _lib.check(l.mage_gemm(C.byref(d), s), l)
             es, ys = a.element_size(), y.element_size()
             nb = float(M) * K * es + float(N) * K * es + float(M) * N * ys
+            if ad is not None and key.startswith("attn_proj_kernel"):
+                nb += 2.0 * M * K * es
             if key == "conv3x3_c64_kernel":
                 nb = float(M) * 64 * es * (0.25 if a_half else 1.0) + float(N) * K * es + float(M) * N * ys
             if residual is not None:
@@ -348,6 +357,21 @@
               kv_outer_stride, kv_axis_stride, causal=False, kv_len=None, kv_len_div=1, scale=None, out_split: int = 0,
               drop_p: float = 0.0, drop_seed: int = 0, split_kind: int = 0, o_outer_stride: int = 0, o_axis_stride: int = 0):
     l, s = _dev(q)
+    d = _attn_desc(q, k, v, out, ldq=ldq, ldk=ldk, ldv=ldv, ldo=ldo, n_seq=n_seq, inner=inner, nq=nq, nk=nk, n_head=n_head,
+                   q_outer_stride=q_outer_stride, q_axis_stride=q_axis_stride, kv_outer_stride=kv_outer_stride, kv_axis_stride=kv_axis_stride,
+                   causal=causal, kv_len=kv_len, kv_len_div=kv_len_div, scale=scale, out_split=out_split, drop_p=drop_p, drop_seed=drop_seed,
+                   split_kind=split_kind, o_outer_stride=o_outer_stride, o_axis_stride=o_axis_stride)
+    ev = PROFILE.begin() if PROFILE.wants("attention") else None
+    _lib.check(l.mage_attention(C.byref(d), s), l)
+    if ev is not None:
+        es = q.element_size()
+        PROFILE.end("attention", ev, 4.0 * n_seq * nq * nk * n_head * 32, float(n_seq) * n_head * 32 * es * (2 * nq + 2 * nk))
+    return out
+
+
+def _attn_desc(q, k, v, out, *, ldq, ldk, ldv, ldo, n_seq, inner, nq, nk, n_head, q_outer_stride, q_axis_stride,
+               kv_outer_stride, kv_axis_stride, causal=False, kv_len=None, kv_len_div=1, scale=None, out_split: int = 0,
+               drop_p: float = 0.0, drop_seed: int = 0, split_kind: int = 0, o_outer_stride: int = 0, o_axis_stride: int = 0) -> AttnDesc:
     d = AttnDesc()
     d.dtype = split_kind or code(q)
     d.q, d.k, d.v, d.out = q.data_ptr(), k.data_ptr(), v.data_ptr(), out.data_ptr()
@@ -361,12 +385,8 @@
     d.out_split = out_split
     d.drop_p, d.drop_seed = float(drop_p), int(drop_seed) & (2 ** 64 - 1)
     d.o_outer_stride, d.o_axis_stride = o_outer_stride, o_axis_stride
-    ev = PROFILE.begin() if PROFILE.wants("attention") else None
-    _lib.check(l.mage_attention(C.byref(d), s), l)
-    if ev is not None:
-        es = q.element_size()
-        PROFILE.end("attention", ev, 4.0 * n_seq * nq * nk * n_head * 32, float(n_seq) * n_head * 32 * es * (2 * nq + 2 * nk))
-    return out
+    d._keep = kv_len
+    return d
 
 
 def embedding(ids: torch.Tensor, table: torch.Tensor, out: torch.Tensor, *, relu: bool = False, group: Optional[int] = None,
```

After: 5797, median of 6. No clear change (+1.0%).
